# maple3142/gf2bv

Measured on AMD Instinct MI355X. Metric: GF(2) row-XORs/s (solve_one, dense NxN), higher is better.
Workload: dtype u64

## Files before the change

gf2bv_amd/csrc/gf2_kernels.hip.h:

```cpp
#pragma once
#include <hip/hip_runtime.h>
#include <stdint.h>
#include <type_traits>

typedef unsigned long long u64;
typedef long long i64;

#define GF2_GMAX 4
#define GF2_TW 2
#define GF2_TW_LOG 1
#define GF2_LPR 1
#define GF2_OWN_LOG 3
#define GF2_FEW_UNITS 8
#ifndef GF2_BATCH
#define GF2_BATCH 4
#endif
#ifndef GF2_UROWS
#define GF2_UROWS 2
#endif

__device__ __forceinline__ long long tidx(long long row, long long word, long long srows)
{
	return ((word >> GF2_TW_LOG) * srows + row) * GF2_TW + (word & (GF2_TW - 1));
}
struct PanelRec {
	int start;
	int p;
	u64 mask;
};

struct PanelAux {
	int slot_row[64];
	u64 comb[64];
	u64 src_mult[64][GF2_GMAX];
	int first_after;
	int pad;
};

#define GF2_NEVER 0x7f7f7f7f

#define GF2_FEW_MISSING 8
#define GF2_GROUP 16
#define GF2_MAXGROUPS 16

struct SolveState {
	int rank;
	int inconsistent;
	int first;
	unsigned arrive;
	int wide;
	unsigned garr[GF2_MAXGROUPS];
	unsigned claim;
	int self_giveups;
	int fast_off, fast_done;
	int fast_blocks;
	int poison;
	int gate_timeout;
	int fast_pub;
	int sp_chunk;
	int sp_nz;
};

struct SyncFlags {
	int narrow_done;
	int bulk_done;
	unsigned cnt_narrow;
};
struct DoneSignal { unsigned *count; int *flag; int value; };

struct FindUnit {
	u64 have;
	int cnt;
	int first_nonsrc;
	int chunks;
	int pad;
	int srow[64];
	u64 bc[64];
};

__device__ __forceinline__ u64 readlane64(u64 v, int l)
{
	unsigned lo = __builtin_amdgcn_readlane((unsigned)v, l);
	unsigned hi = __builtin_amdgcn_readlane((unsigned)(v >> 32), l);
	return ((u64)hi << 32) | lo;
}
#pragma clang diagnostic push
#pragma clang diagnostic ignored "-Winline-asm"
__device__ __forceinline__ void writelane3(unsigned &d0, unsigned s0, unsigned &d1, unsigned s1, int &d2, int s2, int l)
{
	asm volatile("s_mov_b32 m0, %6\n\tv_writelane_b32 %0, %3, m0\n\tv_writelane_b32 %1, %4, m0\n\tv_writelane_b32 %2, %5, m0"
	             : "+v"(d0), "+v"(d1), "+v"(d2) : "s"(s0), "s"(s1), "s"(s2), "s"(l) : "m0");
}
#pragma clang diagnostic pop
__device__ __forceinline__ int ctz64(u64 v) { return __ffsll((long long)v) - 1; }
__device__ __forceinline__ int uniform(int v) { return __builtin_amdgcn_readfirstlane(v); }
__device__ __forceinline__ u64 lanemask_lt(int lane) { return lane ? (~0ull >> (64 - lane)) : 0ull; }
__device__ __forceinline__ uint4 xor4(uint4 a, uint4 b) { return make_uint4(a.x ^ b.x, a.y ^ b.y, a.z ^ b.z, a.w ^ b.w); }

__host__ __device__ __forceinline__ i64 mult_rows(i64 rows) { return (rows + 63) & ~(i64)63; }
__host__ __device__ __forceinline__ i64 midx(int g, i64 row, i64 rows)
{
	(void)rows;
	return row * 4 + (g ^ (int)((row >> 3) & 1));
}
__device__ __forceinline__ u64 mult_stored(int T, u64 m, i64 row)
{
	(void)T;
	const int sh = 8 * (int)(row & 7);
	return sh ? ((m >> sh) | (m << (64 - sh))) : m;
}
__device__ __forceinline__ u64 mult_plain(int T, u64 v, i64 row)
{
	(void)T;
	const int sh = 8 * (int)(row & 7);
	return sh ? ((v << sh) | (v >> (64 - sh))) : v;
}

struct SysStride { i64 m_words, arena_bytes; };
template <class P>
__device__ __forceinline__ P *sys_at(P *p, i64 bytes)
{
	typedef typename std::remove_cv<P>::type Q;
	return reinterpret_cast<P *>(reinterpret_cast<char *>(const_cast<Q *>(p)) + bytes);
}

__host__ __device__ __forceinline__ i64 owned_item(i64 ct, i64 first, int ulog, int world, int wrank)
{
	if (world <= 1) return first + ct;
	const i64 usz = (i64)1 << ulog;
	const i64 u_first = first >> ulog;
	const i64 u0 = u_first + (((wrank - u_first % world) % world) + world) % world;
	const i64 head = (u0 == u_first) ? usz - (first & (usz - 1)) : 0;
	if (ct < head) return first + ct;
	const i64 c2 = ct - head;
	return ((u0 + ((head ? 1 : 0) + c2 / usz) * world) << ulog) + c2 % usz;
}

__global__ void k_pack_digits(const uint32_t *__restrict__ digits, const i64 *__restrict__ off,
                              int bpd, i64 rows, i64 cols, i64 wtot, i64 srows, u64 *__restrict__ M, SysStride ss, i64 dig_base)
{
	off += blockIdx.z * rows;
	M += blockIdx.z * ss.m_words;
	const i64 w = (i64)blockIdx.x * blockDim.x + threadIdx.x;
	if (w >= wtot) return;
	for (i64 r = blockIdx.y; r < rows; r += gridDim.y) {
	const uint32_t *d = digits + (off[r] - dig_base);
	i64 nd = off[r + 1] - off[r];
	u64 val = 0;
	i64 c0 = w * 64;
	if (c0 < cols) {
		i64 p0 = c0 + 1;
		i64 di = p0 / bpd;
		int sh = (int)(p0 % bpd);
		int filled = 0;
		while (filled < 64 && di < nd) {
			u64 piece = (u64)(d[di] >> sh);
			val |= piece << filled;
			filled += bpd - sh;
			sh = 0;
			di++;
		}
		if (cols - c0 < 64) val &= (1ull << (cols - c0)) - 1;
	}
	if (w == (cols >> 6) && nd > 0) val |= (u64)(d[0] & 1u) << (cols & 63);
	M[tidx(r, w, srows)] = val;
	}
}

__global__ void __launch_bounds__(256)
k_to_tiled(const u64 *__restrict__ src, i64 stride, i64 rows, i64 ntiles, i64 wt, i64 srows, u64 *__restrict__ dst,
           i64 src_sys_words, SysStride ss)
{
	static_assert(GF2_TW == 2, "16-byte tiles");
	src += blockIdx.z * src_sys_words;
	dst += blockIdx.z * ss.m_words;
	__shared__ uint4 buf[16 * 65];
	const int t = threadIdx.x;
	const i64 row0 = (i64)blockIdx.x * 64, tile0 = (i64)blockIdx.y * 16;
	const bool even = ((stride & 1) == 0) && ((reinterpret_cast<size_t>(src) & 15) == 0);
#pragma unroll
	for (int i = 0; i < 4; i++) {
		const int r = (t >> 4) + 16 * i, c = t & 15;
		const i64 row = row0 + r, w = (tile0 + c) * 2;
		uint4 v = make_uint4(0, 0, 0, 0);
		if (row < rows && w < wt) {
			const u64 *p = src + row * stride + w;
			if (even && w + 1 < wt) v = *reinterpret_cast<const uint4 *>(p);
			else {
				const u64 a = p[0], b2 = (w + 1 < wt) ? p[1] : 0ull;
				v = make_uint4((unsigned)a, (unsigned)(a >> 32), (unsigned)b2, (unsigned)(b2 >> 32));
			}
		}
		buf[c * 65 + r] = v;
	}
	__syncthreads();
#pragma unroll
	for (int i = 0; i < 4; i++) {
		const int c = (t >> 6) + 4 * i, r = t & 63;
		const i64 row = row0 + r, tile = tile0 + c;
		if (row < rows && tile < ntiles) reinterpret_cast<uint4 *>(dst)[tile * srows + row] = buf[c * 65 + r];
	}
}


__global__ void __launch_bounds__(256)
k_win_gather(const u64 *__restrict__ M, i64 rows, i64 srows, int j0, int gb, u64 *__restrict__ Wb, const SolveState *__restrict__ st, SysStride ss)
{
	if (sys_at(st, blockIdx.y * ss.arena_bytes)->poison) return;
	M += blockIdx.y * ss.m_words;
	Wb = sys_at(Wb, blockIdx.y * ss.arena_bytes);
	const i64 t = (i64)blockIdx.x * blockDim.x + threadIdx.x;
	const i64 i = t / gb;
	const int g = (int)(t % gb);
	if (i >= rows) return;
	Wb[i * GF2_GMAX + g] = M[tidx(i, j0 + g, srows)];
}

__global__ void __launch_bounds__(256)
k_win_scatter(u64 *__restrict__ M, i64 rows, i64 srows, int j0, int gb, const u64 *__restrict__ Wb,
              const int *__restrict__ died, const SolveState *__restrict__ st, SysStride ss)
{
	M += blockIdx.y * ss.m_words;
	Wb = sys_at(Wb, blockIdx.y * ss.arena_bytes);
	died = sys_at(died, blockIdx.y * ss.arena_bytes);
	if (sys_at(st, blockIdx.y * ss.arena_bytes)->poison) return;
	const i64 t = (i64)blockIdx.x * blockDim.x + threadIdx.x;
	const i64 i = t / gb;
	const int g = (int)(t % gb);
	if (i >= rows || died[i] != GF2_NEVER) return;
	M[tidx(i, j0 + g, srows)] = Wb[i * GF2_GMAX + g];
}

#define GF2_ST(ptr, val) __hip_atomic_store((ptr), (val), __ATOMIC_RELAXED, __HIP_MEMORY_SCOPE_AGENT)
#define GF2_LD(ptr) __hip_atomic_load((ptr), __ATOMIC_RELAXED, __HIP_MEMORY_SCOPE_AGENT)

#define GF2_GATE_TICKS 500000000ull
__global__ void k_probe_wait(int *flag, int *result, unsigned long long ticks)
{
	const unsigned long long t0 = wall_clock64();
	int ok = 0;
	while (!(ok = GF2_LD(flag)) && wall_clock64() - t0 < ticks) __builtin_amdgcn_s_sleep(2);
	*result = ok ? 1 : 2;
}
__global__ void k_probe_set(int *flag) { GF2_ST(flag, 1); }
__global__ void __launch_bounds__(512) k_probe_hold_bulk(unsigned long long *stamp, unsigned long long ticks)
{
	__shared__ unsigned big[133 * 256];
	big[threadIdx.x] = threadIdx.x;
	__syncthreads();
	const unsigned long long t0 = wall_clock64();
	if (blockIdx.x == 0 && threadIdx.x == 0) *stamp = t0;
	while (wall_clock64() - t0 < ticks) __builtin_amdgcn_s_sleep(8);
	if (big[(threadIdx.x + 1) & 511] == 0xffffffffu) *stamp = 0;
}
__global__ void __launch_bounds__(256) k_probe_panel_work(unsigned long long *stamp, unsigned long long ticks)
{
	__shared__ unsigned mid[23 * 256];
	mid[threadIdx.x] = threadIdx.x;
	__syncthreads();
	const unsigned long long t0 = wall_clock64();
	while (wall_clock64() - t0 < ticks) __builtin_amdgcn_s_sleep(4);
	if (threadIdx.x == 0) *stamp = wall_clock64();
	if (mid[(threadIdx.x + 1) & 255] == 0xffffffffu) *stamp = 0;
}
__global__ void __launch_bounds__(256) k_probe_stamp_panel(unsigned long long *stamp)
{
	__shared__ unsigned mid[23 * 256];
	mid[threadIdx.x] = threadIdx.x;
	__syncthreads();
	if (threadIdx.x == 0) *stamp = wall_clock64();
	if (mid[(threadIdx.x + 1) & 255] == 0xffffffffu) *stamp = 0;
}
__global__ void __launch_bounds__(64)
k_probe_xcc(int *out)
{
	if (threadIdx.x == 0) out[blockIdx.x] = (int)(__builtin_amdgcn_s_getreg(20 | (0 << 6) | (3 << 11)) & 15u);
}
__global__ void __launch_bounds__(64)
k_gate(SyncFlags *__restrict__ sf, SolveState *__restrict__ st, int set_narrow, int set_bulk, int need_narrow, int need_bulk,
       SysStride ss)
{
	sf = sys_at(sf, blockIdx.y * ss.arena_bytes); st = sys_at(st, blockIdx.y * ss.arena_bytes);
	if (threadIdx.x != 0) return;
	if (set_narrow > 0) GF2_ST(&sf->narrow_done, set_narrow);
	if (set_bulk > 0) GF2_ST(&sf->bulk_done, set_bulk);
	const unsigned long long t0 = wall_clock64();
	int polls = 0;
	while (GF2_LD(&sf->narrow_done) < need_narrow || GF2_LD(&sf->bulk_done) < need_bulk) {
		if (++polls < 512) __builtin_amdgcn_s_sleep(2); else __builtin_amdgcn_s_sleep(64);
		if (wall_clock64() - t0 > GF2_GATE_TICKS || GF2_LD(&st->gate_timeout)) { GF2_ST(&st->gate_timeout, 1); break; }
	}
}
__device__ __forceinline__ void signal_light(DoneSignal sig, i64 arena_off, unsigned total_wgs)
{
	if (!sig.count) return;
	asm volatile("s_waitcnt vmcnt(0)" ::: "memory");
	__builtin_amdgcn_fence(__ATOMIC_RELEASE, "workgroup");
	__syncthreads();
	if (threadIdx.x == 0) {
		unsigned *cnt = sys_at(sig.count, arena_off);
		const unsigned old = __hip_atomic_fetch_add(cnt, 1u, __ATOMIC_RELAXED, __HIP_MEMORY_SCOPE_AGENT);
		if (old + 1 == total_wgs) { GF2_ST(cnt, 0u); GF2_ST(sys_at(sig.flag, arena_off), sig.value); }
	}
}

#ifdef GF2_STEP_PROBE
#define GF2_PROBE_WGS 384
#define GF2_PROBE_UNITS 256
__device__ int gf2_probe_j0 = -1;
__device__ unsigned long long gf2_probe_wg[GF2_GMAX + 1][GF2_PROBE_WGS][4];
__device__ unsigned long long gf2_probe_un[GF2_GMAX + 1][GF2_PROBE_UNITS][6];
__device__ unsigned long long gf2_probe_gj[4];
__device__ unsigned long long gf2_probe_fast[32];
__device__ unsigned long long gf2_probe_upd[GF2_PROBE_WGS][6];
__device__ unsigned long long gf2_probe_wave[5][16];
#define GF2_PROBE_WG(k) do { if (probe_on && threadIdx.x == 0 && blockIdx.x < GF2_PROBE_WGS) gf2_probe_wg[probe_step][blockIdx.x][k] = wall_clock64(); } while (0)
#define GF2_PROBE_UN(k) do { if (gf2_probe_on_u && lane == 0 && u < GF2_PROBE_UNITS) gf2_probe_un[gf2_probe_step_u][u][k] = wall_clock64(); } while (0)
#define GF2_PROBE_UNV(k, v) do { if (gf2_probe_on_u && lane == 0 && u < GF2_PROBE_UNITS) gf2_probe_un[gf2_probe_step_u][u][k] = (v); } while (0)
#else
#define GF2_PROBE_WG(k) do { } while (0)
#define GF2_PROBE_UN(k) do { } while (0)
#define GF2_PROBE_UNV(k, v) do { } while (0)
#endif

struct FindState {
	u64 bw, bc, have;
	int nslots;
	bool colslots;
	int srow;
};

__device__ __forceinline__ unsigned wave_or32(unsigned x)
{
	x |= (unsigned)__builtin_amdgcn_update_dpp(0, (int)x, 0x111, 0xf, 0xf, false);
	x |= (unsigned)__builtin_amdgcn_update_dpp(0, (int)x, 0x112, 0xf, 0xf, false);
	x |= (unsigned)__builtin_amdgcn_update_dpp(0, (int)x, 0x114, 0xf, 0xf, false);
	x |= (unsigned)__builtin_amdgcn_update_dpp(0, (int)x, 0x118, 0xf, 0xf, false);
	x |= (unsigned)__builtin_amdgcn_update_dpp(0, (int)x, 0x142, 0xa, 0xf, false);
	x |= (unsigned)__builtin_amdgcn_update_dpp(0, (int)x, 0x143, 0xc, 0xf, false);
	return (unsigned)__builtin_amdgcn_readlane((int)x, 63);
}
__device__ __forceinline__ u64 wave_or(u64 v)
{
	return ((u64)wave_or32((unsigned)(v >> 32)) << 32) | wave_or32((unsigned)v);
}
__device__ __forceinline__ unsigned wave_xor32(unsigned x)
{
	x ^= (unsigned)__builtin_amdgcn_update_dpp(0, (int)x, 0x111, 0xf, 0xf, false);
	x ^= (unsigned)__builtin_amdgcn_update_dpp(0, (int)x, 0x112, 0xf, 0xf, false);
	x ^= (unsigned)__builtin_amdgcn_update_dpp(0, (int)x, 0x114, 0xf, 0xf, false);
	x ^= (unsigned)__builtin_amdgcn_update_dpp(0, (int)x, 0x118, 0xf, 0xf, false);
	x ^= (unsigned)__builtin_amdgcn_update_dpp(0, (int)x, 0x142, 0xa, 0xf, false);
	x ^= (unsigned)__builtin_amdgcn_update_dpp(0, (int)x, 0x143, 0xc, 0xf, false);
	return (unsigned)__builtin_amdgcn_readlane((int)x, 63);
}
__device__ __forceinline__ u64 wave_xor(u64 v)
{
	return ((u64)wave_xor32((unsigned)(v >> 32)) << 32) | wave_xor32((unsigned)v);
}

template <class IDX>
__device__ __forceinline__ u64 xor_over_bits(const u64 *base, u64 bits, IDX idx)
{
	u64 acc = 0;
	while (bits) {
		const int b0 = ctz64(bits); bits &= bits - 1;
		const u64 h1 = bits ? ~0ull : 0ull; const int b1 = bits ? ctz64(bits) : b0; bits &= bits - 1;
		const u64 h2 = bits ? ~0ull : 0ull; const int b2 = bits ? ctz64(bits) : b0; bits &= bits - 1;
		const u64 h3 = bits ? ~0ull : 0ull; const int b3 = bits ? ctz64(bits) : b0; bits &= bits - 1;
		const u64 v0 = base[idx(b0)], v1 = base[idx(b1)], v2 = base[idx(b2)], v3 = base[idx(b3)];
		acc ^= v0 ^ (v1 & h1) ^ (v2 & h2) ^ (v3 & h3);
	}
	return acc;
}

__device__ __forceinline__ u64 xor_and64(u64 x, u64 v, unsigned m)
{
	const unsigned lo = (unsigned)__builtin_amdgcn_bitop3_b32((int)(unsigned)x, (int)(unsigned)v, (int)m, 0x78);
	const unsigned hi = (unsigned)__builtin_amdgcn_bitop3_b32((int)(unsigned)(x >> 32), (int)(unsigned)(v >> 32), (int)m, 0x78);
	return ((u64)hi << 32) | lo;
}
template <bool HI>
__device__ __forceinline__ unsigned halfbit_mask(u64 x, int bb)
{
	return (unsigned)__builtin_amdgcn_sbfe((int)(unsigned)(HI ? (x >> 32) : x), (unsigned)bb, 1u);
}

template <int K>
__device__ __forceinline__ u64 transpose_stage(u64 x, int lane)
{
	constexpr u64 mk = K == 32 ? 0x00000000ffffffffull : K == 16 ? 0x0000ffff0000ffffull : K == 8 ? 0x00ff00ff00ff00ffull
	                 : K == 4 ? 0x0f0f0f0f0f0f0f0full : K == 2 ? 0x3333333333333333ull : 0x5555555555555555ull;
	auto partner = [&](unsigned v) -> unsigned {
		if (K == 1) return (unsigned)__builtin_amdgcn_update_dpp(0, (int)v, 0xb1, 0xf, 0xf, false);
		if (K == 2) return (unsigned)__builtin_amdgcn_update_dpp(0, (int)v, 0x4e, 0xf, 0xf, false);
		if (K == 8) return (unsigned)__builtin_amdgcn_update_dpp(0, (int)v, 0x128, 0xf, 0xf, false);
		if (K == 4) {
			const int a = __builtin_amdgcn_update_dpp(0, (int)v, 0x104, 0xf, 0x5, false);
			return (unsigned)__builtin_amdgcn_update_dpp(a, (int)v, 0x114, 0xf, 0xa, false);
		}
		return (unsigned)__builtin_amdgcn_ds_bpermute((lane ^ K) << 2, (int)v);
	};
	const u64 pv = ((u64)partner((unsigned)(x >> 32)) << 32) | partner((unsigned)x);
	return (lane & K) ? ((x & ~mk) | ((pv >> K) & mk)) : ((x & mk) | ((pv << K) & ~mk));
}
__device__ __forceinline__ u64 wave_transpose64(u64 x, int lane)
{
	x = transpose_stage<32>(x, lane); x = transpose_stage<16>(x, lane); x = transpose_stage<8>(x, lane);
	x = transpose_stage<4>(x, lane); x = transpose_stage<2>(x, lane); x = transpose_stage<1>(x, lane);
	return x;
}

__device__ __forceinline__ u64 gj_columns(FindState &S, u64 w, int row, int lane)
{
#ifdef GF2_STEP_PROBE
	const bool gjp = gf2_probe_j0 >= 0 && blockIdx.x == 0 && blockIdx.y == 0 && threadIdx.x == 0;
	if (gjp) gf2_probe_gj[0] = wall_clock64();
#endif
	u64 col = wave_transpose64(w, lane);
#ifdef GF2_STEP_PROBE
	if (gjp) gf2_probe_gj[1] = wall_clock64();
#endif
	u64 used = 0, have = 0;
	int Lv = 0;
	for (int b = 0; b < 64; b++) {
		const u64 v = readlane64(col, b);
		const u64 a = v & ~used;
		if (!a) continue;
		const int L = ctz64(a);
		used |= 1ull << L; have |= 1ull << b;
		const u64 vm = v & ~(1ull << L);
		const unsigned mk = 0u - (unsigned)((col >> L) & 1);
		col = xor_and64(col, vm, mk);
		unsigned clo = (unsigned)col, chi = (unsigned)(col >> 32);
		writelane3(clo, (unsigned)v, chi, (unsigned)(v >> 32), Lv, L, b);
		col = ((u64)chi << 32) | clo;
	}
#ifdef GF2_STEP_PROBE
	if (gjp) gf2_probe_gj[2] = wall_clock64();
#endif
	const u64 rows_t = wave_transpose64(col, lane);
// ... 1362 lines not shown
		comb[g] = aux[j0 + gc].comb[r];
#pragma unroll
		for (int e = 0; e < GF2_GMAX; e++) smul[g][e] = (e < g) ? aux[j0 + gc].src_mult[r][e] : 0ull;
		mrow[g] = multset[midx(gc, ic, rows)];
		if (g >= gb) { rec[g].p = 0; rec[g].mask = 0; mrow[g] = 0; }
	}
	u64 wv[W];
#pragma unroll
	for (int e = 0; e < W; e++) wv[e] = M[tidx(ic, wlo + (e < gnext ? e : 0), srows)];
	const int my_died = wmask ? died[ic] : 0;
	if (blockIdx.x != 0 && (i64)(blockIdx.x + 1) * 256 <= first) {
		if (wmask && (t & 63) == 0 && (i >> 6) < mask_words) { wmask[i >> 6] = 0; wmask[mask_words + (i >> 6)] = 0; }
		return;
	}
	int anyp = 0;
#pragma unroll
	for (int g = 0; g < GF2_GMAX; g++) anyp |= rec[g].p;
	if (anyp) {
#pragma unroll
		for (int g = 0; g < GF2_GMAX; g++) {
			const u64 v = M[tidx(r < rec[g].p ? srow[g] : 0, wlo + (live ? w : 0), srows)];
			S[(g * 64 + r) * W + w] = (r < rec[g].p && live) ? v : 0ull;
			if (w == 0 && ((rec[g].mask >> r) & 1)) Bk[g * 64 + __popcll(rec[g].mask & lanemask_lt(r))] = r;
		}
		__syncthreads();
		auto build_tables = [&](const u64 *rows64) {
			const int n = t >> 4, v = t & 15;
			u64 a[W] = { 0, 0, 0, 0 };
#pragma unroll
			for (int k = 0; k < 4; k++) {
				const u64 on = ((v >> k) & 1) ? ~0ull : 0ull;
#pragma unroll
				for (int e = 0; e < W; e++) a[e] ^= rows64[(4 * n + k) * W + e] & on;
			}
#pragma unroll
			for (int e = 0; e < W; e++) Tn[(n * 16 + v) * W + e] = a[e];
		};
#pragma unroll
		for (int g = 0; g < GF2_GMAX; g++) {
			if (g >= gb) break;
			build_tables(&S[g * 64 * W]);
			__syncthreads();
			if (!((rec[g].mask >> r) & 1)) Pbit[(g * 64 + r) * W + w] = 0;
			if (r < rec[g].p) {
				const u64 acc = nibble_word(Tn, comb[g], w);
				Pbit[(g * 64 + Bk[g * 64 + r]) * W + w] = acc;
				if (blockIdx.x == 0 && live) Uwin[(i64)(rec[g].start + r) * GF2_GMAX + w] = acc;
			}
			__syncthreads();
			build_tables(&Pbit[g * 64 * W]);
			__syncthreads();
#pragma unroll
			for (int h = g + 1; h < GF2_GMAX; h++)
				if (h < gb && r < rec[h].p) S[(h * 64 + r) * W + w] ^= nibble_word(Tn, smul[h][g], w);
			if (i < rows && mrow[g]) {
				u64 acc[W];
				nibble_rows(Tn, mult_plain(upd_T, mrow[g], ic), acc);
#pragma unroll
				for (int e = 0; e < W; e++) wv[e] ^= acc[e];
			}
			__syncthreads();
		}
	}
	if (wmask) {
		u64 any = 0;
#pragma unroll
		for (int e = 0; e < W; e++) if (e < gnext) any |= wv[e];
		const bool alive = i < rows && my_died == GF2_NEVER;
		const u64 ba = __ballot(alive), bn = __ballot(alive && any != 0);
		if ((t & 63) == 0 && (i >> 6) < mask_words) { wmask[i >> 6] = ba; wmask[mask_words + (i >> 6)] = bn; }
	}
	if (i >= rows) return;
#pragma unroll
	for (int e = 0; e < W; e++)
		if (e < gnext) Wb_out[i * GF2_GMAX + e] = wv[e];
}

__global__ void __launch_bounds__(256)
k_window_masks(const u64 *__restrict__ Wb, i64 rows, int gb, const int *__restrict__ died, u64 *__restrict__ wmask, const SolveState *__restrict__ st, SysStride ss)
{
	{
		const i64 ao = blockIdx.y * ss.arena_bytes;
		Wb = sys_at(Wb, ao); died = sys_at(died, ao); wmask = sys_at(wmask, ao); st = sys_at(st, ao);
	}
	if (st->poison) return;
	const i64 mask_words = (rows + 63) >> 6;
	const i64 i = (i64)blockIdx.x * 256 + threadIdx.x, ic = i < rows ? i : rows - 1;
	u64 any = 0;
	for (int e = 0; e < gb; e++) any |= Wb[ic * GF2_GMAX + e];
	const bool alive = i < rows && died[ic] == GF2_NEVER;
	const u64 ba = __ballot(alive), bn = __ballot(alive && any != 0);
	if ((threadIdx.x & 63) == 0 && (i >> 6) < mask_words) { wmask[i >> 6] = ba; wmask[mask_words + (i >> 6)] = bn; }
}

__global__ void __launch_bounds__(256)
k_unwind(u64 *__restrict__ M, i64 srows, int G, int npanels, int nblocks, const SolveState *__restrict__ st,
         const int *__restrict__ pivcol, const int *__restrict__ urow, const u64 *__restrict__ Uwin, int world, int wrank,
         int tl_K, int tl_bend, SysStride ss)
{
	{
		const i64 ao = blockIdx.y * ss.arena_bytes;
		M += blockIdx.y * ss.m_words;
		st = sys_at(st, ao); pivcol = sys_at(pivcol, ao); urow = sys_at(urow, ao); Uwin = sys_at(Uwin, ao);
	}
	const i64 t = (i64)blockIdx.x * blockDim.x + threadIdx.x;
	const i64 k = t / GF2_GMAX;
	const int e = (int)(t % GF2_GMAX);
	if (k >= st->rank) return;
	const int b = (pivcol[k] >> 6) / G;
	if (b + 1 >= nblocks) return;
	if (tl_K > 0 && b < tl_bend && (b + 1) % tl_K == 0) return;
	const int wlo = (b + 1) * G;
	const int gnext = (npanels - wlo < G) ? npanels - wlo : G;
	if (world > 1 && ((wlo + e) >> GF2_OWN_LOG) % world != wrank) return;
	if (e < gnext) M[tidx(urow[k], wlo + e, srows)] = Uwin[k * GF2_GMAX + e];
}

struct SlabSeg { const void *src; void *dst; unsigned bytes; };
struct SlabSegs { SlabSeg s[5]; };
__global__ void __launch_bounds__(256)
k_slab_copy(SlabSegs segs)
{
	const size_t tid = (size_t)blockIdx.x * blockDim.x + threadIdx.x, nth = (size_t)gridDim.x * blockDim.x;
#pragma unroll
	for (int k = 0; k < 5; k++) {
		const SlabSeg g = segs.s[k];
		if (!g.bytes) continue;
		if (((g.bytes | (unsigned)(size_t)g.src | (unsigned)(size_t)g.dst) & 15u) == 0) {
			const uint4 *a = static_cast<const uint4 *>(g.src); uint4 *b = static_cast<uint4 *>(g.dst);
			for (size_t i = tid; i < g.bytes / 16; i += nth) b[i] = a[i];
		} else {
			const unsigned *a = static_cast<const unsigned *>(g.src); unsigned *b = static_cast<unsigned *>(g.dst);
			for (size_t i = tid; i < g.bytes / 4; i += nth) b[i] = a[i];
		}
	}
}

__global__ void __launch_bounds__(256)
k_import_marks(int j0, int gb, const PanelRec *__restrict__ panels, const PanelAux *__restrict__ aux,
               int *__restrict__ died, int *__restrict__ pivcol, int *__restrict__ urow)
{
	const int g = threadIdx.x >> 6, lane = threadIdx.x & 63;
	if (g >= gb) return;
	const PanelRec rec = panels[j0 + g];
	if ((rec.mask >> lane) & 1) pivcol[rec.start + __popcll(rec.mask & lanemask_lt(lane))] = 64 * (j0 + g) + lane;
	if (lane < rec.p) {
		const int sr = aux[j0 + g].slot_row[lane];
		urow[rec.start + lane] = sr;
		died[sr] = j0 + g;
	}
}


template <int TW, int WPW>
__global__ void __launch_bounds__(64 * WPW)
k_block_trsm(u64 *__restrict__ M, i64 srows, int j0, int gb, int wlo, int group_begin, int world, int wrank,
             const PanelRec *__restrict__ panels, const PanelAux *__restrict__ aux, int nw_lo, int nw_hi, u64 *__restrict__ Pc,
             SysStride ss)
{
	__builtin_amdgcn_s_setprio(2);
	M += blockIdx.y * ss.m_words;
	panels = sys_at(panels, blockIdx.y * ss.arena_bytes);
	aux = sys_at(aux, blockIdx.y * ss.arena_bytes);
	if (Pc) Pc = sys_at(Pc, blockIdx.y * ss.arena_bytes);
	constexpr int NT = 64 * WPW;
	static_assert(WPW == 4 && NT == 256, "thread <-> table entry mapping below");
	__shared__ u64 S[GF2_GMAX * 64 * WPW];
	__shared__ u64 Pbit[GF2_GMAX * 64 * WPW];
	__shared__ u64 Tn[16 * 16 * WPW];
	__shared__ int Bk[GF2_GMAX * 64];
	const i64 w0 = owned_item(blockIdx.x, group_begin, GF2_OWN_LOG - 2, world, wrank) * WPW;
	const int t = threadIdx.x;
	const int r = t / WPW, w = t % WPW;
	auto at = [&](i64 row) -> u64 & { return M[tidx(row, w0 + w, srows)]; };
	const bool live = w0 + w >= wlo && !(w0 + w >= nw_lo && w0 + w < nw_hi);
	PanelRec rec[GF2_GMAX];
	int srow[GF2_GMAX];
	u64 comb[GF2_GMAX], smul[GF2_GMAX][GF2_GMAX];
#pragma unroll
	for (int g = 0; g < GF2_GMAX; g++) {
		const int gc = g < gb ? g : 0;
		rec[g] = panels[j0 + gc];
		srow[g] = aux[j0 + gc].slot_row[r];
		comb[g] = aux[j0 + gc].comb[r];
#pragma unroll
		for (int e = 0; e < GF2_GMAX; e++) smul[g][e] = (e < g) ? aux[j0 + gc].src_mult[r][e] : 0ull;
		if (g >= gb) { rec[g].p = 0; rec[g].mask = 0; }
	}
#pragma unroll
	for (int g = 0; g < GF2_GMAX; g++) {
		const u64 v = at(r < rec[g].p ? srow[g] : 0);
		S[(g * 64 + r) * WPW + w] = (r < rec[g].p && live) ? v : 0ull;
		Pbit[(g * 64 + r) * WPW + w] = 0;
		if (w == 0 && ((rec[g].mask >> r) & 1)) Bk[g * 64 + __popcll(rec[g].mask & lanemask_lt(r))] = r;
	}
	__syncthreads();
	auto build_tables = [&](const u64 *rows64) {
		const int n = t >> 4, v = t & 15;
		u64 a[WPW] = { 0, 0, 0, 0 };
#pragma unroll
		for (int k = 0; k < 4; k++) {
			const u64 on = ((v >> k) & 1) ? ~0ull : 0ull;
#pragma unroll
			for (int e = 0; e < WPW; e++) a[e] ^= rows64[(4 * n + k) * WPW + e] & on;
		}
#pragma unroll
		for (int e = 0; e < WPW; e++) Tn[(n * 16 + v) * WPW + e] = a[e];
	};
	auto lookup = [&](u64 m) {
		u64 acc = 0;
#pragma unroll
		for (int n = 0; n < 16; n++) {
			const unsigned half = n < 8 ? (unsigned)m : (unsigned)(m >> 32);
			acc ^= Tn[(n * 16 + ((half >> (4 * (n & 7))) & 15u)) * WPW + w];
		}
		return acc;
	};
#pragma unroll
	for (int g = 0; g < GF2_GMAX; g++) {
		if (g >= gb) break;
		build_tables(&S[g * 64 * WPW]);
		__syncthreads();
		if (r < rec[g].p) {
			const u64 acc = lookup(comb[g]);
			Pbit[(g * 64 + Bk[g * 64 + r]) * WPW + w] = acc;
			if (live) at(srow[g]) = acc;
		}
		if (g + 1 >= gb) break;
		__syncthreads();
		build_tables(&Pbit[g * 64 * WPW]);
		__syncthreads();
#pragma unroll
		for (int h = g + 1; h < GF2_GMAX; h++)
			if (h < gb && r < rec[h].p) S[(h * 64 + r) * WPW + w] ^= lookup(smul[h][g]);
		__syncthreads();
	}
	if (Pc) {
		__syncthreads();
		const i64 wabs = w0 + w;
#pragma unroll
		for (int g = 0; g < GF2_GMAX; g++)
			Pc[(((wabs >> 1) * GF2_GMAX + g) * 64 + r) * 2 + (wabs & 1)] = Pbit[(g * 64 + r) * WPW + w];
	}
	(void)NT;
}

__host__ __device__ __forceinline__ int mult_slot(int g, i64 row) { return g ^ (int)((row >> 3) & 1); }
__host__ __device__ __forceinline__ u64 mult_rot(u64 m, i64 row)
{
	const int sh = 8 * (int)(row & 7);
	return sh ? ((m >> sh) | (m << (64 - sh))) : m;
}
__host__ __device__ __forceinline__ u64 mult_unrot(u64 m, i64 row)
{
	const int sh = 8 * (int)(row & 7);
	return sh ? ((m << sh) | (m >> (64 - sh))) : m;
}

typedef unsigned u32x4 __attribute__((ext_vector_type(4)));
typedef __attribute__((address_space(3))) const u32x4 *lds_u4_ptr;

template <int NT, bool HALF, int DEPTH, bool PIPE, int LB, bool STREAM = false>
__global__ void __launch_bounds__(LB)
k_update16(u64 *__restrict__ M, i64 rows, i64 srows, int j0, int gb, int wlo,
           const PanelRec *__restrict__ panels, const PanelAux *__restrict__ aux,
           const u64 *__restrict__ mult4, const int *__restrict__ blk_first,
           int tile_begin, int ntiles, int world, int wrank, const uint4 *__restrict__ Pc, SysStride ss, int xcd_nsys)
{
	unsigned bx = blockIdx.x, gx = gridDim.x, by = blockIdx.y;
	if (xcd_nsys > 0) {
		const unsigned slot = bx >> 3, xcd = bx & 7;
		gx = gx / (unsigned)xcd_nsys;
		by = (slot / gx) * 8 + xcd;
		bx = slot % gx;
	}
	{
		const i64 ao = (i64)by * ss.arena_bytes;
		M += (i64)by * ss.m_words;
		panels = sys_at(panels, ao); aux = sys_at(aux, ao); mult4 = sys_at(mult4, ao); blk_first = sys_at(blk_first, ao);
		if (Pc) Pc = sys_at(Pc, ao);
	}
	constexpr int NW = NT / 64;
	__shared__ __attribute__((aligned(256))) uint4 tab[2 * 256 * 16];
	__shared__ uint4 stage[GF2_GMAX * 64];
	__shared__ int prow[GF2_GMAX * 64];
	const int lane = threadIdx.x & 63, wv = threadIdx.x >> 6;
	if ((unsigned)(size_t)tab != 0u) __builtin_trap();

	int anyp = 0;
	for (int g = 0; g < gb; g++) anyp |= panels[j0 + g].p;
	if (!anyp) return;
	const i64 rlo = (i64)(*blk_first) & ~(i64)63;
	const i64 R64 = (rows + 63) & ~(i64)63;
	constexpr int ALIGN = NW * 64;
	const i64 R = (R64 - rlo + ALIGN - 1) / ALIGN * ALIGN;
	const i64 total = (i64)ntiles * R;
	i64 chunk = (total + gx - 1) / gx;
	chunk = (chunk + ALIGN - 1) / ALIGN * ALIGN;
	i64 pos = (i64)bx * chunk;
	const i64 pend = (pos + chunk < total) ? pos + chunk : total;

	unsigned KC[6];
	{
		const int rq_lo = lane & 7, rq_hi = (lane >> 3) & 1;
#pragma unroll
		for (int v = 0; v < 6; v++) {
			unsigned k = 1u << 24;
#pragma unroll
			for (int b = 0; b < 3; b++) {
				const int s = 3 * v + b;
				if (s < 16) k |= (unsigned)(16 * (8 * ((s >> 3) ^ rq_hi) + (((s & 7) + rq_lo) & 7))) << (8 * b);
			}
			asm volatile("" : "+v"(k));
			KC[v] = k;
		}
	}

	unsigned sgx = 0, sgy = 0, sgz = 0, sgw = 0;
	bool have_staged = false;
	for (bool first_span = true; pos < pend; first_span = false) {
		const int ct = (int)(pos / R);
		const i64 r0 = pos - (i64)ct * R;
		const i64 span = (R - r0 < pend - pos) ? R - r0 : pend - pos;
		pos += span;
		const i64 tile = owned_item(ct, tile_begin, GF2_OWN_LOG - 1, world, wrank);
		const i64 rbeg = rlo + r0;
		if (rbeg >= R64) continue;
		const i64 rend = (rbeg + span < R64) ? rbeg + span : R64;
		uint4 *Mw = reinterpret_cast<uint4 *>(M) + tile * srows;
		const uint4 *mq = reinterpret_cast<const uint4 *>(mult4);
		const i64 nsteps = (rend - rbeg + ALIGN - 1) / ALIGN;
		i64 nb = nsteps;
		if (rbeg + ((nsteps - 1) * NW + wv) * 64 >= rend) nb--;
		struct Bt { uint4 d, m0, m1; i64 row; };
		auto load = [&](Bt &H, i64 i) {
			const i64 ic = i < nb ? i : nb - 1;
			const i64 row = rbeg + (ic * NW + wv) * 64 + lane;
			H.row = row;
			H.m0 = mq[row * 2]; H.m1 = mq[row * 2 + 1];
#ifdef GF2_MB_L2
			H.d = Mw[row & 4095];
#elif defined(GF2_NT_LOAD)
			{ const u32x4 t = __builtin_nontemporal_load(reinterpret_cast<const u32x4 *>(Mw + row)); H.d = make_uint4(t.x, t.y, t.z, t.w); }
#else
			if (STREAM) { const u32x4 t = __builtin_nontemporal_load(reinterpret_cast<const u32x4 *>(Mw + row)); H.d = make_uint4(t.x, t.y, t.z, t.w); }
			else H.d = Mw[row];
#endif
		};
		Bt H[DEPTH] = {};
		if (nb > 0) {
#pragma unroll
			for (int d = 0; d < DEPTH - 1; d++) load(H[d], d);
		}
		if (!first_span) __syncthreads();
		if (first_span && !Pc) {
			for (int t = threadIdx.x; t < GF2_GMAX * 64; t += NT) {
				const int g = t >> 6, b = t & 63;
				int pr = -1;
				if (g < gb) {
					const PanelRec rec = panels[j0 + g];
					if ((rec.mask >> b) & 1) pr = aux[j0 + g].slot_row[__popcll(rec.mask & ((1ull << b) - 1))];
				}
				prow[t] = pr;
			}
			__syncthreads();
		}
		const uint4 *Mq = reinterpret_cast<const uint4 *>(M) + tile * srows;
		if (threadIdx.x < GF2_GMAX * 64) {
			const int pr = Pc ? 0 : prow[threadIdx.x];
			uint4 v;
			if (have_staged) { v.x = sgx; v.y = sgy; v.z = sgz; v.w = sgw; }
			else v = Pc ? Pc[tile * (GF2_GMAX * 64) + threadIdx.x] : Mq[pr >= 0 ? pr : 0];
			const bool k0 = pr >= 0 && 2 * tile >= wlo, k1 = pr >= 0 && 2 * tile + 1 >= wlo;
			if (!k0) { v.x = 0; v.y = 0; }
			if (!k1) { v.z = 0; v.w = 0; }
			stage[threadIdx.x] = v;
		}
		__syncthreads();
		for (int it = threadIdx.x; it < 2 * 31 * 16; it += NT) {
			const int sub = it & 15, e = (it >> 4) % 31, grp = (it >> 4) / 31;
			const int idx = e <= 15 ? e : (e - 15) << 4;
			const uint4 *st = stage + (2 * grp + (sub >> 3)) * 64 + 8 * (sub & 7);
			uint4 acc = make_uint4(0, 0, 0, 0);
			int bits = idx;
			while (bits) {
				const int l = __ffs(bits) - 1; bits &= bits - 1;
				acc = xor4(acc, st[l]);
			}
			tab[grp * 4096 + idx * 16 + sub] = acc;
		}
		__syncthreads();
		for (int it = threadIdx.x; it < 2 * 225 * 16; it += NT) {
			const int sub = it & 15, k = (it >> 4) % 225, grp = (it >> 4) / 225;
			const int lo = 1 + k % 15, hi = (1 + k / 15) << 4;
			uint4 *tb = tab + grp * 4096 + sub;
			tb[(lo | hi) * 16] = xor4(tb[lo * 16], tb[hi * 16]);
		}
		__syncthreads();

		have_staged = false;
		if (pos < pend) {
			const i64 ntile = owned_item((int)(pos / R), tile_begin, GF2_OWN_LOG - 1, world, wrank);
			if (threadIdx.x < GF2_GMAX * 64) {
				uint4 nx;
				if (Pc) nx = Pc[ntile * (GF2_GMAX * 64) + threadIdx.x];
				else {
					const int pr = prow[threadIdx.x];
					nx = (reinterpret_cast<const uint4 *>(M) + ntile * srows)[pr >= 0 ? pr : 0];
				}
				sgx = nx.x; sgy = nx.y; sgz = nx.z; sgw = nx.w;
			}
			have_staged = true;
		}
		auto issue = [&](u32x4 *v, const Bt &H, int r) {
			const unsigned mw[8] = { H.m0.x, H.m0.y, H.m0.z, H.m0.w, H.m1.x, H.m1.y, H.m1.z, H.m1.w };
			const int grp = r >> 1, hf = r & 1;
#pragma unroll
			for (int k = 0; k < 8; k++) {
				const int s = 8 * hf + k;
				const unsigned sel = (unsigned)(s % 3) | ((4u + (unsigned)(k & 3)) << 8) | ((grp ? 3u : 12u) << 16) | (12u << 24);
				const unsigned at = __builtin_amdgcn_perm(mw[2 * (2 * grp + hf) + (k >> 2)], KC[s / 3], sel);
				v[k] = *(lds_u4_ptr)(size_t)at;
			}
		};
		auto fold = [&](uint4 &acc, const u32x4 *v) {
#pragma unroll
			for (int h = 0; h < 4; h++) {
				acc.x = __builtin_amdgcn_bitop3_b32(acc.x, v[2 * h].x, v[2 * h + 1].x, 0x96);
				acc.y = __builtin_amdgcn_bitop3_b32(acc.y, v[2 * h].y, v[2 * h + 1].y, 0x96);
				acc.z = __builtin_amdgcn_bitop3_b32(acc.z, v[2 * h].z, v[2 * h + 1].z, 0x96);
				acc.w = __builtin_amdgcn_bitop3_b32(acc.w, v[2 * h].w, v[2 * h + 1].w, 0x96);
			}
		};
		auto store = [&](const Bt &H, const uint4 &acc) {
#ifdef GF2_MB_L2
			const i64 q = H.row & 4095;
#else
			const i64 q = H.row;
#endif
			if (HALF) reinterpret_cast<u64 *>(Mw + q)[1] = ((u64)acc.w << 32) | acc.z;
#ifdef GF2_NT_STORE
			else { const u32x4 t = { acc.x, acc.y, acc.z, acc.w }; __builtin_nontemporal_store(t, reinterpret_cast<u32x4 *>(Mw + q)); }
#else
			else if (STREAM) { const u32x4 t = { acc.x, acc.y, acc.z, acc.w }; __builtin_nontemporal_store(t, reinterpret_cast<u32x4 *>(Mw + q)); }
			else Mw[q] = acc;
#endif
		};
		if (nb > 0) {
			u32x4 va[8], vb[8];
#ifndef GF2_MB_NOLOOKUP
			if (PIPE) issue(va, H[0], 0);
#endif
			for (i64 i = 0; i < nb; i += DEPTH) {
#pragma unroll
				for (int d = 0; d < DEPTH; d++) {
					if (i + d >= nb) break;
					load(H[(d + DEPTH - 1) % DEPTH], i + d + DEPTH - 1);
					Bt &C = H[d];
					uint4 acc = C.d;
#ifdef GF2_MB_NOLOOKUP
					acc.x ^= C.m0.x ^ C.m0.y ^ C.m0.z ^ C.m0.w; acc.y ^= C.m1.x ^ C.m1.y ^ C.m1.z ^ C.m1.w;
#else
					if (PIPE) {
						issue(vb, C, 1); fold(acc, va);
						issue(va, C, 2); fold(acc, vb);
						issue(vb, C, 3); fold(acc, va);
						issue(va, H[(d + 1) % DEPTH], 0); fold(acc, vb);
					} else {
#pragma unroll
						for (int r = 0; r < 4; r++) { issue(va, C, r); fold(acc, va); }
					}
#endif
					store(C, acc);
				}
			}
		}
	}
}


#ifndef GF2_KMAX
#define GF2_KMAX 12
#endif
#ifndef GF2_KSEG
#define GF2_KSEG 16
#endif

template <int WPW, bool IDENT>
__global__ void __launch_bounds__(64 * WPW)
k_outer_trsm(u64 *__restrict__ M, i64 rows, i64 srows, int j0, int npan, int group_begin,
             const PanelRec *__restrict__ panels, const PanelAux *__restrict__ aux,
             const u64 *__restrict__ mult, i64 set_words, int set0, int nsets, int upd_T, u64 *__restrict__ Tm, SysStride ss)
{
	static_assert(WPW == 4, "thread <-> table entry mapping below");
	{
		const i64 ao = blockIdx.y * ss.arena_bytes;
		M += blockIdx.y * ss.m_words;
		panels = sys_at(panels, ao); aux = sys_at(aux, ao); mult = sys_at(mult, ao); Tm = sys_at(Tm, ao);
	}
	constexpr int NP = GF2_KMAX * GF2_GMAX;
	__shared__ u64 S[NP * 64 * WPW];
	__shared__ u64 Pb[64 * WPW];
	__shared__ u64 Tn[16 * 16 * WPW];
	__shared__ int srowL[NP * 64];
	__shared__ int Bk[64];
	__shared__ u64 mL[NP * 64];
	const i64 w0 = ((i64)group_begin + blockIdx.x) * WPW;
	const int t = threadIdx.x, r = t / WPW, w = t % WPW;
	for (int q = w; q < npan; q += WPW) srowL[q * 64 + r] = (r < panels[j0 + q].p) ? aux[j0 + q].slot_row[r] : -1;
	__syncthreads();
	for (int q = 0; q < npan; q++) {
		const int sr = srowL[q * 64 + r];
		if (IDENT) S[(q * 64 + r) * WPW + w] = (sr >= 0 && q == (int)w0 + w) ? (1ull << r) : 0ull;
		else S[(q * 64 + r) * WPW + w] = sr >= 0 ? M[tidx(sr, w0 + w, srows)] : 0ull;
	}
	auto put_T = [&](int q, u64 v) {
		const i64 i = (i64)q * 64 + r;
		Tm[((i64)blockIdx.x * (NP * 64) + i) * GF2_GMAX + (w ^ (int)((i >> 3) & 1))] = mult_stored(upd_T, v, i);
	};
	auto build_tables = [&](const u64 *rows64) {
		const int n = t >> 4, v = t & 15;
		u64 a[WPW] = { 0, 0, 0, 0 };
#pragma unroll
		for (int k = 0; k < 4; k++) {
			const u64 on = ((v >> k) & 1) ? ~0ull : 0ull;
#pragma unroll
			for (int e = 0; e < WPW; e++) a[e] ^= rows64[(4 * n + k) * WPW + e] & on;
		}
#pragma unroll
		for (int e = 0; e < WPW; e++) Tn[(n * 16 + v) * WPW + e] = a[e];
	};
	auto lookup = [&](u64 m) {
		u64 acc = 0;
#pragma unroll
		for (int n = 0; n < 16; n++) {
			const unsigned half = n < 8 ? (unsigned)m : (unsigned)(m >> 32);
			acc ^= Tn[(n * 16 + ((half >> (4 * (n & 7))) & 15u)) * WPW + w];
		}
		return acc;
	};
	constexpr int MPT = NP * 64 / (64 * WPW);
	u64 mreg[MPT];
	auto fetch_mults = [&](int q) {
		const int g = q % GF2_GMAX, blk = q / GF2_GMAX;
		const u64 *mset = mult + (i64)((set0 + blk) % nsets) * set_words;
#pragma unroll
		for (int u = 0; u < MPT; u++) {
			const int i = t + u * 64 * WPW;
			u64 m = 0;
			if (i < (npan - q - 1) * 64) {
				const int q2 = q + 1 + i / 64, sl = i % 64;
				const int row2 = srowL[q2 * 64 + sl];
				if (row2 >= 0) m = (q2 / GF2_GMAX == blk) ? aux[j0 + q2].src_mult[sl][g] : mult_plain(upd_T, mset[midx(g, row2, rows)], row2);
			}
			mreg[u] = m;
		}
	};
	auto put_mults = [&](int q) {
#pragma unroll
		for (int u = 0; u < MPT; u++) {
			const int i = t + u * 64 * WPW;
			if (i < (npan - q - 1) * 64) mL[(q + 1 + i / 64) * 64 + i % 64] = mreg[u];
		}
	};
	fetch_mults(0);
	put_mults(0);
	__syncthreads();
	for (int q = 0; q < npan; q++) {
		const PanelRec rec = panels[j0 + q];
		if (q + 1 < npan) fetch_mults(q + 1);
		if (rec.p != 0) {
			const u64 comb = aux[j0 + q].comb[r];
			build_tables(&S[q * 64 * WPW]);
			Pb[r * WPW + w] = 0;
			if (w == 0 && ((rec.mask >> r) & 1)) Bk[__popcll(rec.mask & lanemask_lt(r))] = r;
			__syncthreads();
			u64 acc = 0;
			if (r < rec.p) {
				acc = lookup(comb);
				Pb[Bk[r] * WPW + w] = acc;
				if (!IDENT) M[tidx(srowL[q * 64 + r], w0 + w, srows)] = acc;
			}
			if (IDENT) put_T(q, acc);
			__syncthreads();
			if (q + 1 >= npan) break;
			build_tables(Pb);
			__syncthreads();
			for (int q2 = q + 1; q2 < npan; q2++) {
				const u64 m = mL[q2 * 64 + r];
				if (m) S[(q2 * 64 + r) * WPW + w] ^= lookup(m);
			}
		} else if (IDENT) put_T(q, 0ull);
		__syncthreads();
		if (q + 1 < npan) put_mults(q + 1);
		__syncthreads();
	}
}

#define GF2_OUTER_LISTS (2 * GF2_KMAX * GF2_GMAX * 64 + GF2_KMAX)
__global__ void __launch_bounds__(256)
k_outer_prow(int j0, int nblk, const PanelRec *__restrict__ panels, const PanelAux *__restrict__ aux, int *__restrict__ out, SysStride ss)
{
	{
		const i64 ao = blockIdx.y * ss.arena_bytes;
		panels = sys_at(panels, ao); aux = sys_at(aux, ao); out = sys_at(out, ao);
	}
	constexpr int NQ = GF2_KMAX * GF2_GMAX * 64;
	__shared__ int anyb[GF2_KMAX];
	if (threadIdx.x < GF2_KMAX) anyb[threadIdx.x] = 0;
	__syncthreads();
	for (int t = threadIdx.x; t < NQ; t += blockDim.x) {
		int pr = -1, sr = -1;
		if (t < nblk * GF2_GMAX * 64) {
			const int q = t >> 6, b = t & 63;
			const PanelRec rec = panels[j0 + q];
			if ((rec.mask >> b) & 1) { pr = aux[j0 + q].slot_row[__popcll(rec.mask & ((1ull << b) - 1))]; anyb[q / GF2_GMAX] = 1; }
			if (b < rec.p) sr = aux[j0 + q].slot_row[b];
		}
		out[t] = pr;
		out[NQ + GF2_KMAX + t] = sr;
	}
	__syncthreads();
	if (threadIdx.x < GF2_KMAX) out[NQ + threadIdx.x] = anyb[threadIdx.x];
}

template <int SEG, int NT_, int RB, int NB>
__device__ __forceinline__ void
update16k_body(u64 *__restrict__ M, i64 rows, i64 srows, int nblk, const int *__restrict__ gprow,
               const u64 *__restrict__ mult, i64 set_words, int set0, int nsets,
               const int *__restrict__ blk_first, const int *__restrict__ died, int j_end, int tile_begin, int ntiles, SysStride ss,
               int chunk_major)
// ... 2610 lines not shown
```

gf2bv_amd/csrc/gf2_solver.hip:

```cpp
#include "gf2_kernels.hip.h"
#include <hip/hip_ext.h>
#include "../../include/gf2bv_hip.h"

#include <algorithm>
#include <array>
#include <atomic>
#include <chrono>
#include <cstdio>
#include <cstdlib>
#include <cstring>
#include <functional>
#include <map>
#include <memory>
#include <new>
#include <mutex>
#include <string>
#include <thread>
#include <unordered_map>
#include <vector>

namespace {

thread_local std::string g_err = "";

// ... 269 lines not shown
		std::lock_guard<std::mutex> lk(mu);
		auto &v = events[{device, timing ? 1 : 0}];
		if (v.size() < 8192) v.push_back(e); else (void)hipEventDestroy(e);
	}
	hipError_t stream(hipStream_t *s, int device, int cls)
	{
		const bool low = cls & 1;
		{
			std::lock_guard<std::mutex> lk(mu);
			auto &v = streams[{device, cls}];
			if (!v.empty()) { *s = v.back(); v.pop_back(); return hipSuccess; }
		}
		if (!low) return hipStreamCreateWithFlags(s, hipStreamNonBlocking);
		int lo = 0, hi = 0;
		(void)hipDeviceGetStreamPriorityRange(&lo, &hi);
		return hipStreamCreateWithPriority(s, hipStreamNonBlocking, lo);
	}
	void release_stream(hipStream_t s, int device, int cls)
	{
		if (!s) return;
		std::lock_guard<std::mutex> lk(mu);
		streams[{device, cls}].push_back(s);
	}
	static constexpr int kMaxLow = 10;
	std::mutex probe_mu;
	std::map<std::pair<hipStream_t, hipStream_t>, int> pair_ok;
	std::map<int, int> low_created;
	int pairs_probed = 0, pairs_bad = 0;
	hipError_t probe_pair(hipStream_t a, hipStream_t b, int device, int *ok, const Knobs &kn, int depth = 0)
	{
		*ok = 1;
		constexpr int NB = 6;
		unsigned long long *q = nullptr, hq[2 * NB + 2];
		int *fl = nullptr;
		hipError_t e = alloc((void **)&q, sizeof hq, device);
		if (e != hipSuccess) return e;
		struct Free { Pool *p; void *q; ~Free() { p->release(q); } } g1{ this, q };
		if ((e = alloc((void **)&fl, sizeof(int) * 2 * NB, device)) != hipSuccess) return e;
		Free g2{ this, fl };
		if ((e = hipMemsetAsync(fl, 0, sizeof(int) * 2 * NB, a)) != hipSuccess) return e;
		if ((e = hipMemsetAsync(q, 0, sizeof hq, a)) != hipSuccess) return e;
		if ((e = hipStreamSynchronize(a)) != hipSuccess) return e;
		if ((e = hipStreamSynchronize(b)) != hipSuccess) return e;
		int cus = 256;
		(void)hipDeviceGetAttribute(&cus, hipDeviceAttributeMultiprocessorCount, device);
		k_probe_stamp_panel<<<dim3(1), dim3(256), 0, a>>>(q + 2 * NB);
		for (int i = 0; i < NB; i++) {
			k_probe_panel_work<<<dim3(1), dim3(256), 0, a>>>(q + 2 * i, 1000ull);
			k_probe_panel_work<<<dim3(1), dim3(256), 0, a>>>(q + 2 * i + 1, 1000ull);
			k_probe_set<<<dim3(1), dim3(1), 0, a>>>(fl + i);
			k_probe_wait<<<dim3(1), dim3(1), 0, b>>>(fl + i, fl + NB + i, 200000ull);
			k_probe_hold_bulk<<<dim3((unsigned)cus), dim3(512), 0, b>>>(q + 2 * NB + 1, 4000ull);
		}
		if ((e = hipGetLastError()) != hipSuccess) return e;
		if ((e = hipStreamSynchronize(a)) != hipSuccess) return e;
		if ((e = hipStreamSynchronize(b)) != hipSuccess) return e;
		if ((e = hipMemcpy(hq, q, sizeof hq, hipMemcpyDeviceToHost)) != hipSuccess) return e;
		const double chain_us = ((double)hq[2 * NB - 1] - (double)hq[2 * NB]) / 100.0;
		*ok = chain_us < 37.0 * NB;
		if (depth < 2 && chain_us > 0.75 * 37.0 * NB && chain_us < 1.5 * 37.0 * NB) {
			int again = 1;
			if (probe_pair(a, b, device, &again, kn, depth + 1) == hipSuccess) *ok = *ok || again;
		}
		if (kn.trace)
			fprintf(stderr, "[gf2bv trace] stream pair %p / %p: the panel chain of %d probe blocks took %.1f us (%s)\n", (void *)a, (void *)b, NB, chain_us,
			        *ok ? "good" : "waits for the bulk stream");
		return hipSuccess;
	}
	hipError_t low_stream_for(const Knobs &kn, hipStream_t a, int device, hipStream_t *out, int cls = 1, const std::vector<hipStream_t> &also = {})
	{
		if (!(kn.stream_pairs >= 0 ? kn.stream_pairs != 0 : !kn.plain) || !a) return stream(out, device, cls);
		std::lock_guard<std::mutex> pl(probe_mu);
		std::vector<hipStream_t> rejected, with;
		with.push_back(a);
		for (hipStream_t x : also) if (x && x != a) with.push_back(x);
		hipError_t err = hipSuccess;
		*out = nullptr;
		auto known = [&](hipStream_t c) {
			int r = 1;
			for (hipStream_t x : with) {
				auto it = pair_ok.find({x, c});
				if (it == pair_ok.end()) r = r == 0 ? 0 : -1; else if (it->second == 0) r = 0;
			}
			return r;
		};
		for (int attempt = 0; attempt < kMaxLow + 2 && !*out; attempt++) {
			hipStream_t c = nullptr;
			bool known_good = false;
			{
				std::lock_guard<std::mutex> lk(mu);
				auto &v = streams[{device, cls}];
				for (size_t i = v.size(); i-- > 0 && !c;)
					if (known(v[i]) == 1) { c = v[i]; v.erase(v.begin() + (ptrdiff_t)i); known_good = true; }
				for (size_t i = v.size(); i-- > 0 && !c;)
					if (known(v[i]) == -1) { c = v[i]; v.erase(v.begin() + (ptrdiff_t)i); }
				if (!c) {
					if (low_created[device] >= kMaxLow) break;
					low_created[device]++;
				}
			}
			if (known_good) { *out = c; break; }
			if (!c) {
				int lo = 0, hi = 0;
				(void)hipDeviceGetStreamPriorityRange(&lo, &hi);
				if ((err = hipStreamCreateWithPriority(&c, hipStreamNonBlocking, lo)) != hipSuccess) break;
			}
			int all_ok = 1;
			for (hipStream_t x : with) {
				int ok = -1;
				{
					std::lock_guard<std::mutex> lk(mu);
					auto it = pair_ok.find({x, c});
					if (it != pair_ok.end()) ok = it->second;
				}
				if (ok < 0) {
					ok = 1;
					if (probe_pair(x, c, device, &ok, kn) != hipSuccess) { (void)hipGetLastError(); ok = 1; }
					else {
						std::lock_guard<std::mutex> lk(mu);
						pair_ok[{x, c}] = ok;
						pairs_probed++; pairs_bad += !ok;
					}
				}
				if (!ok) { all_ok = 0; break; }
			}
			if (all_ok) *out = c; else rejected.push_back(c);
		}
		if (!*out && !rejected.empty()) { *out = rejected.front(); rejected.erase(rejected.begin()); }
		for (hipStream_t r : rejected) release_stream(r, device, cls);
		if (!*out && err == hipSuccess) return stream(out, device, cls);
		return err;
	}
};
Pool &pool()
{
	static Pool *p = new Pool();
	return *p;
}
int alloc_or_nomem(void **out, size_t bytes, int device, const char *nomem, const char *what)
{
	const hipError_t e = pool().alloc(out, bytes, device);
	if (e == hipErrorOutOfMemory) { (void)hipGetLastError(); return fail(GF2BV_ERR_NOMEM, nomem); }
	if (e != hipSuccess) return fail(GF2BV_ERR_HIP, what, e);
	return GF2BV_OK;
}

int streams_run_concurrently(const Knobs &kn, int device, hipStream_t a, hipStream_t b, int *ok);
int xcd_dispatch_is_round_robin(int device, hipStream_t st, int *ok);
void forget_concurrency(int device);

struct UpdateImpl {
	int G, T, lds_bytes, threads;
	hipError_t (*update)(dim3, hipStream_t, u64 *, i64, i64, int, int, int, const PanelRec *, const PanelAux *,
	                     const u64 *, const int *, int, int, int, int, int, bool, const uint4 *, SysStride, hipEvent_t, hipEvent_t, int);
};

template <int NT, int DEPTH, bool PIPE, int LB>
hipError_t launch_update16(dim3 grid, hipStream_t s, u64 *M, i64 rows, i64 srows, int j0, int gb, int wlo,
                           const PanelRec *panels, const PanelAux *aux, const u64 *multset, const int *blk_first,
                           int tile_begin, int ntiles, int world, int wrank, int nw_lo, bool stream_rows, const uint4 *Pc, SysStride ss,
                           hipEvent_t begun, hipEvent_t done, int xcd_nsys)
{
	if (xcd_nsys > 0) grid = dim3(grid.x * grid.y);
	{
		if (stream_rows && NT == 512 && DEPTH == 3 && PIPE && LB == 512) {
			if (nw_lo < 0)
				hipExtLaunchKernelGGL((k_update16<512, true, 3, true, 512, true>), grid, dim3(512), 0, s, begun, done, 0, M, rows, srows, j0, gb, wlo,
				                      panels, aux, multset, blk_first, tile_begin, ntiles, world, wrank, Pc, ss, xcd_nsys);
			else
				hipExtLaunchKernelGGL((k_update16<512, false, 3, true, 512, true>), grid, dim3(512), 0, s, begun, done, 0, M, rows, srows, j0, gb, wlo,
				                      panels, aux, multset, blk_first, tile_begin, ntiles, world, wrank, Pc, ss, xcd_nsys);
			return hipGetLastError();
		}
	}
	if (nw_lo < 0)
		hipExtLaunchKernelGGL((k_update16<NT, true, DEPTH, PIPE, LB>), grid, dim3(NT), 0, s, begun, done, 0, M, rows, srows, j0, gb, wlo,
		                      panels, aux, multset, blk_first, tile_begin, ntiles, world, wrank, Pc, ss, xcd_nsys);
	else
		hipExtLaunchKernelGGL((k_update16<NT, false, DEPTH, PIPE, LB>), grid, dim3(NT), 0, s, begun, done, 0, M, rows, srows, j0, gb, wlo,
		                      panels, aux, multset, blk_first, tile_begin, ntiles, world, wrank, Pc, ss, xcd_nsys);
	return hipGetLastError();
}
#define UPDATE16_IMPL(NT, D, P, LB) { 4, 8, 2 * 256 * 256 + GF2_GMAX * 64 * 20, NT, launch_update16<NT, D, P, LB> }

const UpdateImpl kUpdates[] = {
	UPDATE16_IMPL(512, 3, true, 512),
	UPDATE16_IMPL(768, 2, true, 768),
	UPDATE16_IMPL(768, 2, true, 1024),
	UPDATE16_IMPL(1024, 2, false, 1024),
	UPDATE16_IMPL(768, 3, true, 768),
	UPDATE16_IMPL(640, 2, true, 640),
};

static_assert(sizeof kUpdates / sizeof kUpdates[0] == Knobs::kNumUpdates, "GF2BV_UPDATE indexes this table");

constexpr int YK = 5, YTW = 16, YNT = 1024;
hipError_t launch_ysweep(dim3 grid, hipStream_t s, u64 *Y, i64 ys, i64 rows, const PanelRec *rec,
                         const u64 *mult, int ntiles, int rpb)
{
	constexpr int lds = SweepCfg<YK, YTW>::LDS_BYTES;
	static std::mutex attr_mu;
	static std::map<int, bool> attr_set;
	int dev = 0;
	(void)hipGetDevice(&dev);
	{
		std::lock_guard<std::mutex> lk(attr_mu);
		if (!attr_set[dev]) {
			hipError_t e = hipFuncSetAttribute((const void *)k_sweep<YK, YTW, YNT>,
			                                   hipFuncAttributeMaxDynamicSharedMemorySize, lds);
			if (e != hipSuccess) return e;
			attr_set[dev] = true;
		}
	}
	k_sweep<YK, YTW, YNT><<<grid, dim3(YNT), lds, s>>>(Y, ys, rows, rec, 1, mult, 0, ntiles, rpb);
	return hipGetLastError();
}

constexpr int TW = GF2_TW;

inline size_t round256(size_t bytes) { return (bytes + 255) & ~(size_t)255; }

struct ArenaLayout {
	size_t st = 0, sf = 0, panels = 0, aux = 0, fu = 0, died = 0, pivcol = 0, urow = 0, blk_first = 0, mult = 0, Wb = 0, Uwin = 0, Pfast = 0,
	       oprow = 0, Tm = 0, Pc = 0, wmask = 0, stride = 0;
};

struct SolverPlan {
	int device = 0;
	i64 rows = 0, cols = 0, stride = 0;
	i64 ntiles = 0, srows = 0;
	int nsys = 1;
	int gang_nsys = 1;
	int world = 1, wrank = 0;
	i64 m_stride = 0, src_sys_words = 0;
	ArenaLayout lay;
	bool view = false;
	bool own_bs = true;
	SysStride ss() const { return SysStride{ m_stride, (i64)lay.stride }; }
	int mode = 0;
	int nrhs = 1;
	bool time_kernels = false;
	Knobs kn;
	const UpdateImpl *impl = nullptr;

	int nsets = 2;
	int tl_K = 0, tl_bend = 0;
	i64 tile_hi = 0;
	static constexpr int nlist = 2;
	bool bulk_waits_outer = false;
	bool ends_outer_panel(int b) const { return tl_K > 0 && b < tl_bend && (b + 1) % tl_K == 0; }
	bool flag_sync = true;
	bool optimistic = true;
	bool xcd_pin = true;
	int sync_base = 0;
	int units = 0;
	bool sparse_on = false;
	int sparse_giveups = 0;
	int sparse_tier = 0;
	int narrow_rpt = 1;
	i64 ys = 0;
	int ny = 0;
	int h_ycol = 0;
	i64 maxr = 0;
	int npanels = 0, nblocks = 0;
	i64 wt = 0, cw = 0;

	std::vector<int> free_order;
	SolveState hst{};
	std::vector<u64> hout;
	std::vector<PanelRec> hp;
	std::vector<int32_t> hpiv;
	std::chrono::steady_clock::time_point t_begin;
	float ms_pack = 0;
};

ArenaLayout arena_layout(const SolverPlan &P)
{
	const i64 R = std::max<i64>(1, P.rows), NP = std::max(1, P.npanels);
	const int G = P.impl->G;
	ArenaLayout L;
	size_t off = 0;
	auto carve = [&](size_t bytes) { size_t at = off; off += round256(bytes); return at; };
	L.st = carve(sizeof(SolveState)); L.sf = carve(sizeof(SyncFlags)); L.panels = carve(sizeof(PanelRec) * NP); L.aux = carve(sizeof(PanelAux) * NP);
	L.fu = carve(sizeof(FindUnit) * (P.units + 1 + GF2_MAXGROUPS)); L.died = carve(sizeof(int) * (size_t)R);
	L.pivcol = carve(sizeof(int) * (P.maxr + 64)); L.urow = carve(sizeof(int) * (P.maxr + 64));
	L.blk_first = carve(sizeof(int) * std::max(1, P.nblocks)); L.mult = carve(sizeof(u64) * P.nsets * G * mult_rows(R) + (P.tl_K ? kOuterSlackBytes : 0));
	L.Wb = carve(sizeof(u64) * 2 * GF2_GMAX * R); L.Uwin = carve(sizeof(u64) * GF2_GMAX * (P.maxr + 64));
	L.Pfast = carve(sizeof(u64) * GF2_GMAX * GF2_GMAX * 64); L.oprow = carve(sizeof(int) * GF2_OUTER_LISTS * P.nlist);
	L.Tm = carve(P.tl_K ? P.nlist * sizeof(u64) * GF2_KMAX * GF2_KMAX * GF2_GMAX * 64 * GF2_GMAX : 0);
	L.Pc = carve(P.kn.pc ? sizeof(u64) * 2 * GF2_GMAX * 64 * (size_t)P.ntiles : 0);
	L.wmask = carve(sizeof(u64) * 2 * (size_t)((R + 63) / 64 + 1));
	L.stride = off;
	return L;
}

struct ArenaPtrs {
	SolveState *st = nullptr;
	SyncFlags *sf = nullptr;
	PanelRec *panels = nullptr;
	PanelAux *aux = nullptr;
	FindUnit *fu = nullptr;
	int *died = nullptr;
	int *pivcol = nullptr, *urow = nullptr, *blk_first = nullptr;
	u64 *mult = nullptr;
	u64 *Wb = nullptr;
	u64 *Uwin = nullptr;
	u64 *Pfast = nullptr;
	int *oprow = nullptr;
	u64 *Tm = nullptr;
	u64 *Pc = nullptr;
	u64 *wmask = nullptr;

	void bind(const ArenaLayout &L, void *arena, bool pc)
	{
		char *base = (char *)arena;
		st = (SolveState *)(base + L.st); sf = (SyncFlags *)(base + L.sf); panels = (PanelRec *)(base + L.panels); aux = (PanelAux *)(base + L.aux);
		fu = (FindUnit *)(base + L.fu); died = (int *)(base + L.died); pivcol = (int *)(base + L.pivcol); urow = (int *)(base + L.urow);
		blk_first = (int *)(base + L.blk_first); mult = (u64 *)(base + L.mult); Wb = (u64 *)(base + L.Wb); Uwin = (u64 *)(base + L.Uwin);
		Pfast = (u64 *)(base + L.Pfast); oprow = (int *)(base + L.oprow); Tm = (u64 *)(base + L.Tm);
		Pc = pc ? (u64 *)(base + L.Pc) : nullptr;
		wmask = (u64 *)(base + L.wmask);
	}
};

struct SolverHandles {
	hipStream_t sA = nullptr, sB = nullptr;
	bool own_sA = false, own_sB = false;
	u64 *M = nullptr;
	bool ext_M = false;
	const u64 *src = nullptr;
	u64 *tmp_src = nullptr;
	u64 *Minv = nullptr;
	u64 *rhs_bad = nullptr;
	void *arena = nullptr;
	hipStream_t sC = nullptr;
	hipEvent_t evOuter = nullptr, evPri = nullptr, evPanelDone = nullptr, evBig = nullptr;
	u64 *Y = nullptr;
	int *ycols = nullptr;
	u64 *out = nullptr;
	hipEvent_t ev0 = nullptr, ev1 = nullptr, ev2 = nullptr, ev3 = nullptr;
	std::vector<hipEvent_t> evA, evPrio, kev, waitPrio;
	hipEvent_t evx = nullptr;
};

struct Solver : SolverPlan, ArenaPtrs, SolverHandles {
	SolverPlan &plan() { return *this; }
	const SolverPlan &plan() const { return *this; }
	Solver() = default;
	Solver(const Solver &) = delete;
	Solver &operator=(const Solver &) = delete;
	~Solver() { release(); }
	void release()
	{
		if (!arena && !M && !tmp_src && !Y && !ycols && !out && !sA && !sB && !ev0) return;
		(void)hipSetDevice(device);
		Pool &P = pool();
		if (view) {
			if (sA && (Y || ycols || out)) (void)hipStreamSynchronize(sA);
			if (own_bs) for (void *p : { (void *)Y, (void *)ycols, (void *)out, (void *)Minv }) P.release(p);
			P.release_event(ev2, true);
			P.release_event(evx, true);
			arena = nullptr; M = nullptr; sA = sB = nullptr; ev0 = ev1 = ev3 = nullptr;
		} else {
			if (sC) (void)hipStreamSynchronize(sC);
			if (sB) (void)hipStreamSynchronize(sB);
			if (arena || M) (void)hipStreamSynchronize(sA);
			for (void *p : { arena, (void *)Y, (void *)ycols, (void *)out, (void *)Minv, (void *)(ext_M ? nullptr : M), (void *)tmp_src }) P.release(p);
			for (hipEvent_t e : { ev0, ev1, ev2, ev3, evx }) P.release_event(e, true);
			for (hipEvent_t e : { evOuter, evPri, evPanelDone, evBig }) P.release_event(e, false);
			if (sC) P.release_stream(sC, device, nsys > 1 ? 3 : 1);
			for (hipEvent_t e : kev) P.release_event(e, true);
			for (hipEvent_t e : evA) P.release_event(e, false);
			for (hipEvent_t e : evPrio) P.release_event(e, false);
			if (own_sB && sB) P.release_stream(sB, device, nsys > 1 ? 3 : 1);
			if (own_sA && sA) P.release_stream(sA, device, false);
		}
		static_cast<ArenaPtrs &>(*this) = ArenaPtrs();
		static_cast<SolverHandles &>(*this) = SolverHandles();
	}
};

}

struct gf2bv_result {
	int status = 0;
	i64 rank = 0, dim = 0, cw = 0;
	std::vector<u64> origin, basis;
	std::vector<int32_t> pivots;
	gf2bv_stats stats{};
};

namespace {

struct Scratch {
	std::vector<void *> bufs;
	std::vector<hipEvent_t> timing_events;
	hipStream_t sync_first = nullptr;
	~Scratch()
	{
		if (sync_first) (void)hipStreamSynchronize(sync_first);
		for (void *p : bufs) pool().release(p);
		for (hipEvent_t e : timing_events) pool().release_event(e, true);
	}
	hipError_t alloc(void **out, size_t bytes, int device)
	{
		hipError_t e = pool().alloc(out, bytes, device);
		if (e == hipSuccess) bufs.push_back(*out);
		return e;
	}
	hipError_t event(hipEvent_t *ev)
	{
		hipError_t e = pool().event(ev, true);
		if (e == hipSuccess) timing_events.push_back(*ev);
		return e;
	}
};

int check_device(int device)
{
	int n = 0;
	hipError_t e = hipGetDeviceCount(&n);
	if (e != hipSuccess || n <= 0)
		return fail(GF2BV_ERR_NODEVICE, "no HIP device visible: gf2bv_amd has no CPU fallback");
	if (device < 0 || device >= n) return fail(GF2BV_ERR_ARG, "device index out of range");
	HIPCHK(hipSetDevice(device));
	return GF2BV_OK;
}

void plan_two_level(Solver &S)
{
	S.tl_K = 0; S.tl_bend = 0; S.nsets = 2;
	if (S.world != 1 || S.ext_M || S.impl->G != GF2_GMAX) return;
	if (S.nsys != 1) return;
	int K = (double)S.rows * (double)S.wt * 8.0 >= 3.0 * 1073741824.0 ? GF2_KMAX : 8;
	double min_bytes = 0.5 * 1073741824.0;
	if (S.kn.two_level == 0) return;
	if (S.kn.two_level > 0) { K = S.kn.two_level; min_bytes = 0; }
	if (S.kn.two_level_min_set) min_bytes = 1048576.0 * S.kn.two_level_min_mib;
	const int G = S.impl->G;
	int bend = 0;
	for (int b0 = 0; b0 + K < S.nblocks; b0 += K) {
		const i64 rows_left = S.rows - (i64)(b0 + K) * 64 * G, words_left = S.wt - (i64)(b0 + K) * G;
		if ((i64)(b0 + K) * 64 * G > S.cols || rows_left <= 0 || words_left <= 0) break;
		if ((double)rows_left * (double)words_left * 8.0 * (double)S.nsys < min_bytes) break;
		bend = b0 + K;
	}
	if (!bend) return;
	S.tl_K = K; S.tl_bend = bend;
	S.nsets = 2 * K;
}

int solver_alloc(Solver &S)
{
	const Knobs &kn = S.kn = Knobs::read();
	S.wt = (S.cols + S.nrhs + 63) / 64;
	S.cw = (S.cols + 63) / 64;
	S.npanels = (int)((S.cols + 63) / 64);
	S.maxr = std::min(S.rows, S.cols);
	S.impl = &kUpdates[S.kn.update];
	S.ntiles = tiles_for(S.wt);
	S.srows = slab_rows(S.rows);
	S.m_stride = S.ntiles * TW * S.srows;
	if (!S.M) HIPCHK(pool().alloc((void **)&S.M, sizeof(u64) * S.m_stride * S.nsys + kOuterSlackBytes, S.device));
	if (S.src && S.rows > 0) {
		k_to_tiled<<<dim3((unsigned)((S.rows + 63) / 64), (unsigned)((S.ntiles + 15) / 16), S.nsys), dim3(256), 0, S.sA>>>(
			S.src, S.stride, S.rows, S.ntiles, std::min(S.wt, S.stride), S.srows, S.M, S.src_sys_words, S.ss());
	}
	const int G = S.impl->G;
	S.nblocks = (S.npanels + G - 1) / G;
	S.tile_hi = S.ntiles;
	plan_two_level(S);
	S.units = (int)std::min<i64>(256, std::max<i64>(1, (S.rows + 255) / 256));
	S.flag_sync = S.world == 1 && !kn.plain && kn.flag_sync != 0 && !kn.serial;
	S.optimistic = kn.optimistic >= 0 ? kn.optimistic != 0 : !kn.plain;
	S.xcd_pin = kn.xcd_pin >= 0 ? kn.xcd_pin != 0 : !kn.plain;
	if (kn.xcd_pin < 0 && !kn.plain && S.nsys >= 8 && S.nsys % 8 == 0) {
		int ok = 0;
		int rc = xcd_dispatch_is_round_robin(S.device, S.sA, &ok);
		if (rc) return rc;
		S.xcd_pin = ok != 0;
	}
	{
		const i64 blocks = (S.rows + 255) / 256 * std::max(1, S.nsys);
		S.narrow_rpt = (int)std::min<i64>(8, std::max<i64>(1, blocks / 256));
	}
	if (kn.serial) { S.sB = S.sA; S.own_sB = false; }
	else {
		if (S.nsys == 1) HIPCHK(pool().low_stream_for(kn, S.sA, S.device, &S.sB));
		else HIPCHK(pool().stream(&S.sB, S.device, 3));
		S.own_sB = true;
	}
	if (S.flag_sync && S.sB != S.sA) {
		int ok = 0;
		int rc = streams_run_concurrently(kn, S.device, S.sA, S.sB, &ok);
		if (rc) return rc;
		S.flag_sync = ok != 0;
	}
	{
		const ArenaLayout &L = S.lay = arena_layout(S);
		S.sync_base = 0;
		HIPCHK(pool().alloc(&S.arena, L.stride * S.nsys, S.device));
		S.bind(L, S.arena, kn.pc);
		for (int s = 0; s < S.nsys; s++) {
			char *b = (char *)S.arena + (size_t)s * L.stride;
			HIPCHK(hipMemsetAsync(b + L.st, 0, L.died - L.st, S.sA));
			HIPCHK(hipMemsetAsync(b + L.died, GF2_NEVER & 0xff, sizeof(int) * (size_t)std::max<i64>(1, S.rows), S.sA));
			HIPCHK(hipMemsetAsync(b + L.blk_first, 0, L.Wb - L.blk_first, S.sA));
		}
	}
	HIPCHK(pool().event(&S.ev0, true));
	HIPCHK(pool().event(&S.ev1, true));
	HIPCHK(pool().event(&S.ev2, true));
	HIPCHK(pool().event(&S.ev3, true));
	if (S.tl_K) {
		for (hipEvent_t *e : { &S.evOuter, &S.evPri, &S.evPanelDone }) HIPCHK(pool().event(e, false));
		if (S.sB != S.sA) { if (S.nsys == 1) HIPCHK(pool().low_stream_for(kn, S.sA, S.device, &S.sC)); else HIPCHK(pool().stream(&S.sC, S.device, 3)); }
		HIPCHK(pool().event(&S.evBig, false));
	}
	S.evA.resize(S.nblocks); S.evPrio.resize(S.nblocks); S.waitPrio.assign(S.nblocks, nullptr);
	for (int b = 0; b < S.nblocks; b++) {
		HIPCHK(pool().event(&S.evA[b], false));
		HIPCHK(pool().event(&S.evPrio[b], false));
	}
	return GF2BV_OK;
}

struct ConcurrencyCache { std::mutex mu; std::map<int, int> known; };
ConcurrencyCache &concurrency_cache() { static ConcurrencyCache c; return c; }
void forget_concurrency(int device)
{
	ConcurrencyCache &c = concurrency_cache();
	std::lock_guard<std::mutex> lk(c.mu);
	c.known[device] = 0;
}
int streams_run_concurrently(const Knobs &kn, int device, hipStream_t a, hipStream_t b, int *ok)
{
	std::mutex &mu = concurrency_cache().mu;
	std::map<int, int> &known = concurrency_cache().known;
	std::lock_guard<std::mutex> lk(mu);
	auto it = known.find(device);
	if (it != known.end()) { *ok = it->second; return GF2BV_OK; }
	if (kn.flag_sync == 2) { *ok = 1; return GF2BV_OK; }
	int *d = nullptr;
	HIPCHK(pool().alloc((void **)&d, 2 * sizeof(int), device));
	struct Free { int *p; ~Free() { pool().release(p); } } guard{d};
	HIPCHK(hipMemsetAsync(d, 0, 2 * sizeof(int), a));
	HIPCHK(hipStreamSynchronize(a));
	HIPCHK(hipStreamSynchronize(b));
	k_probe_wait<<<dim3(1), dim3(1), 0, a>>>(d, d + 1, 200000ull);
	k_probe_set<<<dim3(1), dim3(1), 0, b>>>(d);
	HIPCHK(hipGetLastError());
	HIPCHK(hipStreamSynchronize(a));
	HIPCHK(hipStreamSynchronize(b));
	int h[2] = { 0, 0 };
	HIPCHK(hipMemcpy(h, d, sizeof h, hipMemcpyDeviceToHost));
	*ok = known[device] = (h[1] == 1);
	return GF2BV_OK;
}

int xcd_dispatch_is_round_robin(int device, hipStream_t st, int *ok)
{
	static std::mutex mu;
	static std::map<int, int> known;
	std::lock_guard<std::mutex> lk(mu);
	auto it = known.find(device);
	if (it != known.end()) { *ok = it->second; return GF2BV_OK; }
	int *d = nullptr;
	HIPCHK(pool().alloc((void **)&d, 64 * sizeof(int), device));
	struct Free { int *p; ~Free() { pool().release(p); } } guard{d};
	int h[64];
	int good = 1;
	for (int rep = 0; rep < 2 && good; rep++) {
		k_probe_xcc<<<dim3(64), dim3(64), 0, st>>>(d);
		HIPCHK(hipGetLastError());
		HIPCHK(hipMemcpyAsync(h, d, sizeof h, hipMemcpyDeviceToHost, st));
		HIPCHK(hipStreamSynchronize(st));
		for (int b = 0; b < 64; b++) if (h[b] != h[b & 7]) good = 0;
		for (int a = 0; a < 8; a++) for (int b = a + 1; b < 8; b++) if (h[a] == h[b]) good = 0;
	}
	*ok = known[device] = good;
	return GF2BV_OK;
}

int pick_update_wgs(i64 est_rows, int ntiles, int nsys, int pinned_wgs = 0)
{
	i64 want = 256;
	want = std::max<i64>(1, want / std::max(1, nsys));
	if (pinned_wgs > 0) want = pinned_wgs;
	constexpr i64 min_rows = 2048;
	const i64 cap = std::max<i64>(1, (i64)ntiles * TW / 8 * est_rows / min_rows);
	return (int)std::min(want, cap);
}

i64 owned_count(i64 first, i64 end, int ulog, int world, int wrank)
{
	if (end <= first) return 0;
	if (world <= 1) return end - first;
	i64 n = 0;
	for (i64 u = first >> ulog; u <= (end - 1) >> ulog; u++)
		if (u % world == wrank) n += std::min<i64>(end, (u + 1) << ulog) - std::max<i64>(first, u << ulog);
	return n;
}

int launch_trsm(Solver &S, hipStream_t st, int j0, int gb, int wlo, int nw_lo, int nw_hi)
{
	constexpr int WPW = 4;
	const i64 g0 = wlo / WPW, g1 = S.tile_hi * TW / WPW;
	const i64 ng = owned_count(g0, g1, GF2_OWN_LOG - 2, S.world, S.wrank);
	if (ng <= 0) return GF2BV_OK;
	k_block_trsm<TW, WPW><<<dim3((unsigned)ng, S.nsys), dim3(64 * WPW), 0, st>>>(S.M, S.srows, j0, gb, wlo, (int)g0, S.world, S.wrank,
	                                                                           S.panels, S.aux, nw_lo, nw_hi, S.Pc, S.ss());
	HIPCHK(hipGetLastError());
	return GF2BV_OK;
}

int launch_update_timed(Solver &S, hipStream_t st, int b, int j0, int gb, int wlo, u64 *mset, int tile_begin, int ntiles,
                        int nw_lo, bool last, hipEvent_t *handoff)
{
	hipEvent_t ka = nullptr, kb = nullptr;
	if (S.time_kernels) {
		HIPCHK(pool().event(&ka, true)); HIPCHK(pool().event(&kb, true));
		S.kev.push_back(ka); S.kev.push_back(kb);
	}
	const i64 est_rows = std::max<i64>(256, S.rows - (i64)j0 * 64);
	const bool pin = S.xcd_pin && S.nsys >= 8 && S.nsys % 8 == 0;
	const int wgs = pick_update_wgs(est_rows, ntiles, S.nsys, pin ? S.kn.xcd_wgs : 0);
	const hipEvent_t begun = ka, done = S.time_kernels ? kb : (last && !S.flag_sync ? S.evPrio[b] : nullptr);
	HIPCHK(S.impl->update(dim3((unsigned)wgs, S.nsys), st, S.M, S.rows, S.srows, j0, gb, wlo, S.panels, S.aux, mset,
	                      S.blk_first + b, tile_begin, ntiles, S.world, S.wrank, nw_lo, pin && S.kn.gang_nt,
	                      (const uint4 *)S.Pc, S.ss(), begun, done, pin ? S.nsys : 0));
	if (last && !S.flag_sync) *handoff = done;
	return GF2BV_OK;
}

struct BlockGeom { int j0, gb, wlo, tb, nt_all, gnext; u64 *mset; };
BlockGeom block_geom(const Solver &S, int b)
{
	const int G = S.impl->G;
	BlockGeom g;
	g.j0 = b * G;
	g.gb = std::min(G, S.npanels - g.j0);
	g.wlo = g.j0 + g.gb;
	g.mset = S.mult + (i64)(b % S.nsets) * G * mult_rows(S.rows);
	g.tb = g.wlo / TW;
	g.nt_all = (g.wlo < S.wt) ? (int)S.tile_hi - g.tb : 0;
	g.gnext = (b + 1 < S.nblocks && !S.ends_outer_panel(b)) ? std::min(G, S.npanels - g.wlo) : 0;
	return g;
}

bool fast_block_possible(const Solver &S, const BlockGeom &g)
{
	return S.kn.fast && g.gb == GF2_GMAX && (i64)(g.j0 + g.gb) * 64 <= S.cols && S.rows >= GF2_FAST_NC;
}

int panel_handover(Solver &S, int b)
{
	k_gate<<<dim3(1, S.nsys), dim3(64), 0, S.sA>>>(S.sf, S.st, S.sync_base + b + 1, 0, 0, 0, S.ss());
	HIPCHK(hipGetLastError());
	return GF2BV_OK;
}

constexpr int kSparseByDensity = 2;
int enqueue_block_panel(Solver &S, int b, bool fast_only = false, bool sparse = false)
{
	const BlockGeom g = block_geom(S, b);
	const unsigned row_blocks = (unsigned)((S.rows + 255) / 256);
	u64 *const half[2] = { S.Wb, S.Wb + (i64)GF2_GMAX * S.rows };
	const hipEvent_t done = S.flag_sync ? nullptr : S.evA[b];
	const DoneSignal sig = S.flag_sync ? DoneSignal{ &S.sf->cnt_narrow, &S.sf->narrow_done, S.sync_base + b + 1 } : DoneSignal{};
	if (fast_only && !sparse && S.kn.fused_narrow && S.nsys == 1) {
		const int rpt = (int)std::min<i64>(8, std::max<i64>(S.narrow_rpt, (row_blocks + 127) / 128));
		hipExtLaunchKernelGGL(k_block_fast_narrow, dim3(1 + (row_blocks + rpt - 1) / rpt, S.nsys), dim3(256), 0, S.sA, nullptr, done, 0,
		                      S.M, S.rows, S.srows, g.j0, g.gb, b, (const u64 *)half[0], S.st, S.died, S.panels, S.aux, S.pivcol, S.urow,
		                      S.blk_first + b, S.Pfast, g.mset, S.impl->T, rpt, sig, S.ss());
		HIPCHK(hipGetLastError());
		return GF2BV_OK;
	}
	if (fast_only) {
		if (!sparse)
			k_block_fast<<<dim3(1, S.nsys), dim3(256), 0, S.sA>>>(S.M, S.rows, S.srows, g.j0, g.gb, 1, b, (const u64 *)half[0], S.st, S.died,
			                                                      S.panels, S.aux, S.pivcol, S.urow, S.blk_first + b, S.Pfast, S.ss());
		else if (S.sparse_tier == 0)
			k_block_sparse<256, 4><<<dim3(1, S.nsys), dim3(256), 0, S.sA>>>(S.M, S.rows, S.srows, g.j0, g.gb, 1, b, (const u64 *)half[0], S.st, S.died,
			                                                                 S.panels, S.aux, S.pivcol, S.urow, S.blk_first + b, (const u64 *)S.wmask, S.ss());
		else if (S.sparse_tier == 1)
			k_block_sparse<512, 8><<<dim3(1, S.nsys), dim3(512), 0, S.sA>>>(S.M, S.rows, S.srows, g.j0, g.gb, 1, b, (const u64 *)half[0], S.st, S.died,
			                                                                S.panels, S.aux, S.pivcol, S.urow, S.blk_first + b, (const u64 *)S.wmask, S.ss());
		else
			k_block_sparse<1024, 6><<<dim3(1, S.nsys), dim3(1024), 0, S.sA>>>(S.M, S.rows, S.srows, g.j0, g.gb, 1, b, (const u64 *)half[0], S.st, S.died,
			                                                                  S.panels, S.aux, S.pivcol, S.urow, S.blk_first + b, (const u64 *)S.wmask, S.ss());
		hipExtLaunchKernelGGL(k_narrow_all, dim3((row_blocks + S.narrow_rpt - 1) / S.narrow_rpt, S.nsys), dim3(256), 0, S.sA, nullptr, done, 0,
		                      (const u64 *)S.M, S.rows, S.srows, g.j0, b, (const u64 *)half[0], (const SolveState *)S.st, (const int *)S.died,
		                      (const PanelAux *)S.aux, g.mset, S.impl->T, S.narrow_rpt, sig, S.ss());
		HIPCHK(hipGetLastError());
		return GF2BV_OK;
	}
	if (fast_block_possible(S, g))
		k_block_fast<<<dim3(1, S.nsys), dim3(256), 0, S.sA>>>(S.M, S.rows, S.srows, g.j0, g.gb, 0, b, (const u64 *)half[0], S.st, S.died,
		                                                      S.panels, S.aux, S.pivcol, S.urow, S.blk_first + b, S.Pfast, S.ss());
	for (int s = 0; s <= g.gb; s++) {
		const int gp = s - 1, gf = (s < g.gb) ? s : -1;
		const i64 c0 = (i64)(g.j0 + std::max(gf, 0)) * 64;
		const u64 colmask = (S.cols - c0 >= 64) ? ~0ull : ((1ull << (S.cols - c0)) - 1);
		const int find_wgs = gf >= 0 ? (S.units + 3) / 4 : 0;
		const unsigned wgs = (unsigned)find_wgs + (gp >= 0 ? (row_blocks + S.narrow_rpt - 1) / S.narrow_rpt : 0u);
		const bool ext = !S.flag_sync && s == g.gb && b != S.nblocks - 1;
		hipExtLaunchKernelGGL(k_panel_step, dim3(wgs, S.nsys), dim3(256), 0, S.sA, nullptr, ext ? S.evA[b] : nullptr, 0,
		                      S.M, S.rows, S.srows, g.j0, gp, gf, g.gb, colmask,
		                      (const u64 *)half[s ? (s - 1) & 1 : 0], half[s & 1], S.st, S.died, S.fu, S.units, find_wgs,
		                      S.panels, S.aux, S.pivcol, S.urow, g.mset,
		                      gf == g.gb - 1 ? S.blk_first + b : (int *)nullptr, S.impl->T, kSparseByDensity, S.kn.self_wait_us * 100, S.narrow_rpt, b, S.ss());
	}
	if (b == S.nblocks - 1)
		k_win_scatter<<<dim3((unsigned)((S.rows * g.gb + 255) / 256), S.nsys), dim3(256), 0, S.sA>>>(S.M, S.rows, S.srows, g.j0, g.gb, half[g.gb & 1], S.died, S.st, S.ss());
	HIPCHK(hipGetLastError());
	if (S.flag_sync) { int rc = panel_handover(S, b); if (rc) return rc; }
	else if (b == S.nblocks - 1) HIPCHK(hipEventRecord(S.evA[b], S.sA));
	if (S.kn.debug_sync & 1) HIPCHK(hipDeviceSynchronize());
	return GF2BV_OK;
}

int enqueue_block_bulk(Solver &S, int b)
{
	const BlockGeom g = block_geom(S, b);
	if (S.bulk_waits_outer) { HIPCHK(hipStreamWaitEvent(S.sB, S.evOuter, 0)); S.bulk_waits_outer = false; }
	if (S.flag_sync) {
		k_gate<<<dim3(1, S.nsys), dim3(64), 0, S.sB>>>(S.sf, S.st, 0, S.sync_base + b, S.sync_base + b + 1, 0, S.ss());
		HIPCHK(hipGetLastError());
	} else HIPCHK(hipStreamWaitEvent(S.sB, S.evA[b], 0));
	bool launched = false;
	if (g.nt_all > 0) {
		int rc = launch_trsm(S, S.sB, g.j0, g.gb, g.wlo, g.wlo, g.wlo + g.gnext);
		if (rc) return rc;
		const int wend = g.wlo + g.gnext;
		const int tfull = g.gnext > 0 ? (wend + 1) / 2 : g.wlo / 2;
		const i64 nfull = owned_count(tfull, S.tile_hi, GF2_OWN_LOG - 1, S.world, S.wrank);
		if ((wend & 1) && g.gnext > 0 && owned_count(wend / 2, wend / 2 + 1, GF2_OWN_LOG - 1, S.world, S.wrank) > 0) {
			rc = launch_update_timed(S, S.sB, b, g.j0, g.gb, g.wlo, g.mset, wend / 2, 1, -1, nfull <= 0, &S.waitPrio[b]);
			if (rc) return rc;
			launched = nfull <= 0;
		}
		if (nfull > 0) {
			rc = launch_update_timed(S, S.sB, b, g.j0, g.gb, g.wlo, g.mset, tfull, (int)nfull, 0, true, &S.waitPrio[b]);
			if (rc) return rc;
			launched = true;
		}
	}
	if (!launched && !S.flag_sync) {
		HIPCHK(hipEventRecord(S.evPrio[b], S.sB));
		S.waitPrio[b] = S.evPrio[b];
	}
	if (S.kn.debug_sync & 2) HIPCHK(hipDeviceSynchronize());
	return GF2BV_OK;
}

int enqueue_block_prio(Solver &S, int b)
{
	if (b + 1 >= S.nblocks || S.ends_outer_panel(b)) return GF2BV_OK;
	const BlockGeom g = block_geom(S, b);
	const unsigned row_blocks = (unsigned)((S.rows + 255) / 256);
	if (b > 0 && !S.flag_sync) HIPCHK(hipStreamWaitEvent(S.sA, S.waitPrio[b - 1], 0));
	if (b > 0 && S.flag_sync) {
		k_gate<<<dim3(1, S.nsys), dim3(64), 0, S.sA>>>(S.sf, S.st, 0, 0, 0, S.sync_base + b, S.ss());
		HIPCHK(hipGetLastError());
	}
	k_prio_window<<<dim3(row_blocks, S.nsys), dim3(256), 0, S.sA>>>(S.M, S.rows, S.srows, g.j0, g.gb, g.wlo, std::max(g.gnext, 1),
	                                                             S.panels, S.aux, g.mset, S.blk_first + b, S.Wb, S.Uwin,
	                                                             S.impl->T, S.st, S.ss(), (const int *)S.died, S.sparse_on ? S.wmask : (u64 *)nullptr);
	HIPCHK(hipGetLastError());
	return GF2BV_OK;
}

int enqueue_forward_begin(Solver &S, bool gather_first_window)
{
	HIPCHK(hipEventRecord(S.ev0, S.sA));
	HIPCHK(hipStreamWaitEvent(S.sB, S.ev0, 0));
	if (S.npanels > 0 && gather_first_window) {
		const int g0 = std::min(S.impl->G, S.npanels);
		k_win_gather<<<dim3((unsigned)((S.rows * g0 + 255) / 256), S.nsys), dim3(256), 0, S.sA>>>(S.M, S.rows, S.srows, 0, g0, S.Wb, S.st, S.ss());
	}
	return GF2BV_OK;
}

int enqueue_forward_join(Solver &S)
{
	HIPCHK(hipEventRecord(S.ev3, S.sB));
	HIPCHK(hipStreamWaitEvent(S.sA, S.ev3, 0));
	if (S.nblocks > 1 && S.maxr > 0)
		k_unwind<<<dim3((unsigned)((S.maxr * GF2_GMAX + 255) / 256), S.nsys), dim3(256), 0, S.sA>>>(
			S.M, S.srows, S.impl->G, S.npanels, S.nblocks, S.st, S.pivcol, S.urow, S.Uwin, S.world, S.wrank, S.tl_K, S.tl_bend, S.ss());
	HIPCHK(hipGetLastError());
	return GF2BV_OK;
}

int enqueue_check_rhs(Solver &S)
{
	int g = (int)std::min<i64>(1024, (S.rows + 255) / 256);
	if (S.rhs_bad) {
		const i64 nrw = ((S.cols & 63) + S.nrhs + 63) / 64;
		k_check_rhs_many<<<dim3(g, (unsigned)std::min<i64>(nrw, 65535)), dim3(256), 0, S.sA>>>(S.M, S.rows, S.srows, S.cols, S.nrhs,
		                                                                                      S.died, S.rhs_bad);
	} else {
		k_check_rhs<<<dim3(g, S.nsys), dim3(256), 0, S.sA>>>(S.M, S.rows, S.srows, S.cols, S.died, S.st, S.ss());
	}
	HIPCHK(hipGetLastError());
	HIPCHK(hipEventRecord(S.ev1, S.sA));
	return GF2BV_OK;
}

int enqueue_outer_prepare(Solver &S, hipStream_t st, int b0, int b1)
{
	const int G = S.impl->G;
	const i64 set_words = (i64)G * mult_rows(S.rows);
	const int npan = (b1 - b0) * G;
	int *gprow = S.oprow + (size_t)((b0 / S.tl_K) % S.nlist) * GF2_OUTER_LISTS;
	u64 *Tm = S.Tm + (size_t)((b0 / S.tl_K) % S.nlist) * ((size_t)GF2_KMAX * GF2_KMAX * GF2_GMAX * 64 * GF2_GMAX);
	k_outer_prow<<<dim3(1, S.nsys), dim3(256), 0, st>>>(b0 * G, b1 - b0, S.panels, S.aux, gprow, S.ss());
	if (!S.kn.outer_chain)
		k_outer_trsm<4, true><<<dim3((unsigned)(npan / 4), S.nsys), dim3(256), 0, st>>>(S.M, S.rows, S.srows, b0 * G, npan, 0, S.panels, S.aux, S.mult,
		                                                                               set_words, b0 % S.nsets, S.nsets, S.impl->T, Tm, S.ss());
	HIPCHK(hipGetLastError());
	return GF2BV_OK;
}

int enqueue_outer_apply(Solver &S, hipStream_t st, int b0, int b1, i64 t_begin, i64 t_end)
{
	const int G = S.impl->G;
	const i64 nt = t_end - t_begin;
	if (nt <= 0) return GF2BV_OK;
	const i64 set_words = (i64)G * mult_rows(S.rows);
	int *gprow = S.oprow + (size_t)((b0 / S.tl_K) % S.nlist) * GF2_OUTER_LISTS;
	const int npan = (b1 - b0) * G;
	if (S.kn.outer_chain) {
		const i64 g_begin = t_begin * TW / 4, ng = t_end * TW / 4 - g_begin;
		k_outer_trsm<4, false><<<dim3((unsigned)ng, S.nsys), dim3(256), 0, st>>>(S.M, S.rows, S.srows, b0 * G, npan, (int)g_begin, S.panels, S.aux,
		                                                                          S.mult, set_words, b0 % S.nsets, S.nsets, S.impl->T, (u64 *)nullptr, S.ss());
	} else
		k_outer_apply<<<dim3((unsigned)nt, S.nsys), dim3(512), 0, st>>>(S.M, S.rows, S.srows, b1 - b0, (const int *)gprow,
		                                                                (const u64 *)(S.Tm + (size_t)((b0 / S.tl_K) % S.nlist) * ((size_t)GF2_KMAX * GF2_KMAX * GF2_GMAX * 64 * GF2_GMAX)), (int)t_begin, S.ss());
	HIPCHK(hipGetLastError());
	hipEvent_t ka = nullptr, kb = nullptr;
	if (S.time_kernels) {
		HIPCHK(pool().event(&ka, true)); HIPCHK(pool().event(&kb, true));
		S.kev.push_back(ka); S.kev.push_back(kb);
	}
	const i64 est_lo = std::min<i64>(S.rows, (i64)b0 * 64 * G) & ~(i64)63, R64 = round_up(S.rows, 64);
	constexpr i64 item_rows = (i64)GF2_WSEG * 1024;
	static_assert((size_t)item_rows * 32 <= kOuterSlackBytes, "the slack behind the matrix covers an item");
	const i64 nch = std::max<i64>(1, (R64 - est_lo + item_rows - 1) / item_rows);
	const i64 wgs = std::min<i64>(nch * nt, (i64)1 << 30);
	hipExtLaunchKernelGGL(k_update16k_wide, dim3((unsigned)wgs, S.nsys), dim3(1024), 0, st, ka, kb, 0,
	                      S.M, S.rows, S.srows, b1 - b0, (const int *)gprow, (const u64 *)S.mult,
	                      set_words, b0 % S.nsets, S.nsets, (const int *)(S.blk_first + b0), (const int *)S.died, b1 * G, (int)t_begin, (int)nt, S.ss(), 1);
	HIPCHK(hipGetLastError());
	if (S.kn.debug_sync & 2) HIPCHK(hipDeviceSynchronize());
	return GF2BV_OK;
}

int enqueue_window_gather(Solver &S, int b)
{
	const BlockGeom g = block_geom(S, b);
	k_win_gather<<<dim3((unsigned)((S.rows * g.gb + 255) / 256), S.nsys), dim3(256), 0, S.sA>>>(S.M, S.rows, S.srows, g.j0, g.gb, S.Wb, S.st, S.ss());
	HIPCHK(hipGetLastError());
	return GF2BV_OK;
}

int enqueue_forward(Solver &S)
{
	Trace tr;
	int rc = enqueue_forward_begin(S, true);
	if (rc) return rc;
	bool optimistic = false;
	SolveState hst{};
	const bool may_probe = S.kn.fast && S.optimistic && S.nsys == 1 && S.world == 1 && S.nblocks >= 8 && fast_block_possible(S, block_geom(S, 0));
	auto fast_only_ok = [&](int blk) {
		return fast_block_possible(S, block_geom(S, blk)) && S.rows - (i64)blk * 64 * S.impl->G >= GF2_FAST_NC + 128;
	};
	const bool may_sparse = may_probe && S.kn.sparse_fast && S.tl_K == 0;
	int general_only = -1;
	auto sparse_ok = [&](int blk) { return S.sparse_on && blk != general_only && fast_block_possible(S, block_geom(S, blk)); };
	auto recover = [&](int pb) -> int {
		if (S.sC) HIPCHK(hipStreamSynchronize(S.sC));
		HIPCHK(hipStreamSynchronize(S.sB));
		if (S.tl_K && pb < S.tl_bend) S.tl_bend = pb / S.tl_K * S.tl_K;
		S.bulk_waits_outer = false;
		HIPCHK(hipMemsetAsync(&S.st->poison, 0, sizeof(int), S.sA));
		S.sync_base += S.nblocks + 1;
		return GF2BV_OK;
	};
	int sparse_probes = 1;
	auto one_block = [&](int blk) -> int {
		int r;
		bool sp = sparse_ok(blk);
		if ((r = enqueue_block_panel(S, blk, sp || (optimistic && fast_only_ok(blk)), sp))) return r;
		if (sp && sparse_probes > 0) {
			sparse_probes--;
			HIPCHK(hipMemcpyAsync(&hst, S.st, sizeof hst, hipMemcpyDeviceToHost, S.sA));
			HIPCHK(hipStreamSynchronize(S.sA));
			const int want = hst.sp_nz > 3400 ? 2 : 0;
			if (hst.poison) {
				if ((r = recover(blk))) return r;
				if (++S.sparse_giveups >= 3) S.sparse_on = false; else sparse_probes = 1;
				S.sparse_tier = std::min(2, std::max(S.sparse_tier + 1, want));
				general_only = blk;
				if ((r = enqueue_block_panel(S, blk, false, false))) return r;
			} else S.sparse_tier = std::max(S.sparse_tier, want);
		}
		if ((r = enqueue_block_bulk(S, blk))) return r;
		if ((r = enqueue_block_prio(S, blk))) return r;
		if (blk == 0 && may_probe) {
			HIPCHK(hipMemcpyAsync(&hst, S.st, sizeof hst, hipMemcpyDeviceToHost, S.sA));
			HIPCHK(hipStreamSynchronize(S.sA));
			optimistic = hst.fast_done == 1;
			if (!optimistic && may_sparse && S.nblocks > 1) {
				S.sparse_on = true;
				const BlockGeom g1 = block_geom(S, 1);
				k_window_masks<<<dim3((unsigned)((S.rows + 255) / 256), S.nsys), dim3(256), 0, S.sA>>>((const u64 *)S.Wb, S.rows, g1.gb, (const int *)S.died, S.wmask,
				                                                                                      (const SolveState *)S.st, S.ss());
				HIPCHK(hipGetLastError());
			}
		}
		return GF2BV_OK;
	};
	int b = 0;
	if (S.tl_K) {
		const int G = S.impl->G;
		hipStream_t so = S.sC ? S.sC : S.sB;
		bool big_recorded = false;
		for (int p0 = 0; p0 < S.tl_bend; p0 += S.tl_K) {
			const int p1 = p0 + S.tl_K;
			if (p0 > 0) {
				HIPCHK(hipStreamWaitEvent(S.sA, S.evPri, 0));
				if ((rc = enqueue_window_gather(S, p0))) return rc;
			}
			S.tile_hi = (i64)p1 * G / TW;
			for (b = p0; b < p1; b++)
				if ((rc = one_block(b))) return rc;
			S.tile_hi = S.ntiles;
			if ((rc = enqueue_outer_prepare(S, S.sA, p0, p1))) return rc;
			HIPCHK(hipEventRecord(S.evPanelDone, S.sA));
			HIPCHK(hipStreamWaitEvent(so, S.evPanelDone, 0));
			const i64 t_out = S.ntiles;
			const i64 t0 = (i64)p1 * G / TW, t1 = std::min<i64>(t_out, t0 + (i64)S.tl_K * G / TW);
			const bool side = S.kn.outer_side && S.sB != so && S.sB != S.sA;
			if (side) {
				HIPCHK(hipStreamWaitEvent(S.sB, S.evPanelDone, 0));
				if (big_recorded) HIPCHK(hipStreamWaitEvent(S.sB, S.evBig, 0));
				if ((rc = enqueue_outer_apply(S, S.sB, p0, p1, t0, t1))) return rc;
				HIPCHK(hipEventRecord(S.evPri, S.sB));
				if ((rc = enqueue_outer_apply(S, so, p0, p1, t1, t_out))) return rc;
			} else {
				if ((rc = enqueue_outer_apply(S, so, p0, p1, t0, t1))) return rc;
				HIPCHK(hipEventRecord(S.evPri, so));
				if ((rc = enqueue_outer_apply(S, so, p0, p1, t1, t_out))) return rc;
			}
			HIPCHK(hipEventRecord(S.evBig, so));
			big_recorded = true;
		}
		HIPCHK(hipEventRecord(S.evOuter, so));
		b = S.tl_bend;
		HIPCHK(hipStreamWaitEvent(S.sA, S.evPri, 0));
		if (b < S.nblocks && (rc = enqueue_window_gather(S, b))) return rc;
		S.bulk_waits_outer = S.sC != nullptr;
	}
	for (; b < S.nblocks; b++)
		if ((rc = one_block(b))) return rc;
	if ((rc = enqueue_forward_join(S))) return rc;
	tr.mark(S.kn, "forward: all blocks submitted");
	while (optimistic || S.sparse_on) {
		HIPCHK(hipMemcpyAsync(&hst, S.st, sizeof hst, hipMemcpyDeviceToHost, S.sA));
		HIPCHK(hipStreamSynchronize(S.sA));
		if (!hst.poison) break;
		{
			const int pb = hst.poison - 1;
			if ((rc = recover(pb))) return rc;
			optimistic = false;
			if (S.sparse_on && ++S.sparse_giveups > 3) S.sparse_on = false;
			S.sparse_tier = std::min(2, S.sparse_tier + 1);
			general_only = pb;
			for (b = pb; b < S.nblocks; b++)
				if ((rc = one_block(b))) return rc;
			if ((rc = enqueue_forward_join(S))) return rc;
		}
	}
	return enqueue_check_rhs(S);
}

int enqueue_backward(Solver &S, const std::vector<int> &ycols_host)
{
	S.ny = (int)ycols_host.size();
	const i64 nyw = (S.ny + 63) / 64;
	S.ys = round_up(nyw, YTW);
	HIPCHK(pool().alloc((void **)&S.ycols, sizeof(int) * S.ny, S.device));
	HIPCHK(hipMemcpyAsync(S.ycols, ycols_host.data(), sizeof(int) * S.ny, hipMemcpyHostToDevice, S.sA));
	HIPCHK(pool().alloc((void **)&S.Y, sizeof(u64) * std::max<i64>(1, S.maxr) * S.ys, S.device));
	HIPCHK(hipMemsetAsync(S.Y, 0, sizeof(u64) * std::max<i64>(1, S.maxr) * S.ys, S.sA));
	HIPCHK(pool().alloc((void **)&S.out, sizeof(u64) * S.ny * std::max<i64>(1, S.cw), S.device));
	HIPCHK(hipMemsetAsync(S.out, 0, sizeof(u64) * S.ny * std::max<i64>(1, S.cw), S.sA));
	u64 *bmult = S.mult;
	const int rpb = 2048;
	if (S.maxr > 0) {
		const i64 kchunk = std::max<i64>(1, (1ll << 24) / nyw);
		for (i64 k0 = 0; k0 < S.maxr; k0 += kchunk) {
			const i64 waves = std::min(kchunk, S.maxr - k0) * nyw;
			k_extract_y<<<dim3((unsigned)((waves + 3) / 4)), dim3(256), 0, S.sA>>>(S.M, S.srows, S.st, S.urow, S.pivcol,
			                                                                      S.ycols, S.ny, S.Y, S.ys, k0);
		}
		const int ytiles = (int)(S.ys / YTW);
		for (int q = S.npanels - 1; q >= 1; q--) {
			const i64 bound = std::min<i64>((i64)64 * q, S.maxr);
			int g = (int)std::min<i64>(1024, (bound + 255) / 256);
			k_gather_mult_u<<<dim3(g), dim3(256), 0, S.sA>>>(S.M, S.srows, q, S.panels + q, S.urow, bmult);
			const i64 nrb = (bound + rpb - 1) / rpb;
			HIPCHK(launch_ysweep(dim3((unsigned)(ytiles * nrb)), S.sA, S.Y, S.ys, S.maxr, S.panels + q, bmult, ytiles, rpb));
		}
		for (i64 k0 = 0; k0 < S.maxr; k0 += kchunk << 6) {
			const i64 thr = std::min(kchunk << 6, S.maxr - k0) * nyw;
			k_scatter_solution<<<dim3((unsigned)((thr + 255) / 256)), dim3(256), 0, S.sA>>>(S.Y, S.ys, S.st, S.pivcol, S.ny,
			                                                                              S.out, std::max<i64>(1, S.cw), k0);
		}
	}
	HIPCHK(hipGetLastError());
	HIPCHK(hipEventRecord(S.ev2, S.sA));
	return GF2BV_OK;
}

int enqueue_backward_parity(Solver &S, const std::vector<int> &ycols_host)
{
	S.ny = (int)ycols_host.size();
	const i64 cw = std::max<i64>(1, S.cw);
	HIPCHK(pool().alloc((void **)&S.ycols, sizeof(int) * S.ny, S.device));
	HIPCHK(hipMemcpyAsync(S.ycols, ycols_host.data(), sizeof(int) * S.ny, hipMemcpyHostToDevice, S.sA));
	HIPCHK(pool().alloc((void **)&S.out, sizeof(u64) * S.ny * cw, S.device));
	HIPCHK(hipMemsetAsync(S.out, 0, sizeof(u64) * S.ny * cw, S.sA));
	unsigned char *accv = reinterpret_cast<unsigned char *>(S.mult);
	const i64 nacc = std::max<i64>(1, S.maxr);
	HIPCHK(pool().alloc((void **)&S.Y, sizeof(u64) * 64 * 16 * std::max(1, S.npanels), S.device));
	if (S.npanels > 0)
		k_bs_diag<<<dim3(S.npanels), dim3(256), 0, S.sA>>>(S.M, S.srows, S.npanels, S.panels, S.urow, S.Y, SysStride{0, 0}, (i64)0);
	const int ngroups = (S.npanels + GF2_BSG - 1) / GF2_BSG;
	const bool inv = S.kn.bs_inv >= 0 ? S.kn.bs_inv != 0 && ngroups >= 1 : ngroups >= 16;
	if (inv) {
		HIPCHK(pool().alloc((void **)&S.Minv, sizeof(u64) * (size_t)ngroups * 16 * 64 * 16, S.device));
		static std::mutex mu;
		static std::map<int, bool> raised;
		{
			std::lock_guard<std::mutex> lk(mu);
			if (!raised[S.device]) {
				HIPCHK(hipFuncSetAttribute((const void *)k_bs_inv, hipFuncAttributeMaxDynamicSharedMemorySize, GF2_BSINV_LDS));
				raised[S.device] = true;
			}
		}
		k_bs_inv<<<dim3(ngroups), dim3(1024), GF2_BSINV_LDS, S.sA>>>(S.Y, S.npanels, S.panels, S.pivcol, S.Minv);
	}
	for (int v0 = 0; v0 < S.ny; v0 += GF2_BSV) {
		const int nv = std::min(GF2_BSV, S.ny - v0);
		for (int qb = S.npanels; qb > 0; qb -= GF2_BSG) {
			const int qa = std::max(0, qb - GF2_BSG);
			const int waves = (qb - qa) * 64;
			k_bs_far<<<dim3((waves + 3) / 4), dim3(256), 0, S.sA>>>(S.M, S.srows, cw, qa, qb, S.panels, S.urow, S.pivcol, S.ycols + v0, nv,
			                                                        S.out + (i64)v0 * cw, accv, nacc, SysStride{0, 0}, (i64)0);
			if (inv)
				k_bs_near2<<<dim3(1), dim3(1024), 0, S.sA>>>(cw, qa, qb, S.panels, S.pivcol, nv, S.out + (i64)v0 * cw, accv, nacc, S.Minv,
				                                             (S.npanels - qb) / GF2_BSG);
			else
				k_bs_near<<<dim3(1), dim3(256), 0, S.sA>>>(S.Y, cw, qa, qb, S.panels, S.pivcol, nv, S.out + (i64)v0 * cw, accv, nacc,
				                                           SysStride{0, 0}, (i64)0, (i64)0);
		}
	}
	HIPCHK(hipGetLastError());
	HIPCHK(hipEventRecord(S.ev2, S.sA));
	return GF2BV_OK;
}

int enqueue_backward_gang(Solver &S)
{
	S.ny = 1;
	const i64 cw = std::max<i64>(1, S.cw);
	S.h_ycol = (int)S.cols;
	HIPCHK(pool().alloc((void **)&S.ycols, sizeof(int), S.device));
	HIPCHK(hipMemcpyAsync(S.ycols, &S.h_ycol, sizeof(int), hipMemcpyHostToDevice, S.sA));
	HIPCHK(pool().alloc((void **)&S.out, sizeof(u64) * cw * S.nsys, S.device));
	HIPCHK(hipMemsetAsync(S.out, 0, sizeof(u64) * cw * S.nsys, S.sA));
	unsigned char *accv = reinterpret_cast<unsigned char *>(S.mult);
	const i64 nacc = std::max<i64>(1, S.maxr);
	const i64 dgw = (i64)64 * 16 * std::max(1, S.npanels);
	HIPCHK(pool().alloc((void **)&S.Y, sizeof(u64) * dgw * S.nsys, S.device));
	if (S.npanels > 0)
		k_bs_diag<<<dim3(S.npanels, S.nsys), dim3(256), 0, S.sA>>>(S.M, S.srows, S.npanels, S.panels, S.urow, S.Y, S.ss(), dgw);
	for (int qb = S.npanels; qb > 0; qb -= GF2_BSG) {
		const int qa = std::max(0, qb - GF2_BSG);
		const int waves = (qb - qa) * 64;
		k_bs_far<<<dim3((waves + 3) / 4, S.nsys), dim3(256), 0, S.sA>>>(S.M, S.srows, cw, qa, qb, S.panels, S.urow, S.pivcol, S.ycols, 1,
		                                                                S.out, accv, nacc, S.ss(), cw);
		k_bs_near<<<dim3(1, S.nsys), dim3(256), 0, S.sA>>>(S.Y, cw, qa, qb, S.panels, S.pivcol, 1, S.out, accv, nacc, S.ss(), dgw, cw);
	}
	HIPCHK(hipGetLastError());
	HIPCHK(hipEventRecord(S.ev2, S.sA));
	return GF2BV_OK;
}

int enqueue_backsub(Solver &S, const std::vector<int> &ycols)
{
	if ((i64)ycols.size() <= GF2_BS_MAXRHS && !S.kn.ysweep) return enqueue_backward_parity(S, ycols);
	return enqueue_backward(S, ycols);
}

int solver_enqueue(Solver &S)
{
	Trace tr;
	int rc = solver_alloc(S);
	tr.mark(S.kn, "solver_alloc");
	if (rc) return rc;
	rc = enqueue_forward(S);
	tr.mark(S.kn, "enqueue_forward");
	if (rc) return rc;
	if (S.mode == GF2BV_MODE_SINGLE) return enqueue_backsub(S, { (int)S.cols });
	return GF2BV_OK;
}

std::vector<int> m4ri_free_order(const int32_t *piv, i64 rank, i64 cols)
{
	std::vector<int> order(cols);
	for (i64 i = 0; i < cols; i++) order[i] = (int)i;
	for (i64 i = 0; i < rank; i++) std::swap(order[i], order[piv[i]]);
	return std::vector<int>(order.begin() + rank, order.end());
}

int load_free_order(Solver &S)
{
	HIPCHK(hipMemcpyAsync(&S.hst, S.st, sizeof S.hst, hipMemcpyDeviceToHost, S.sA));
	HIPCHK(hipStreamSynchronize(S.sA));
	std::vector<int32_t> piv(S.hst.rank);
	if (S.hst.rank)
		HIPCHK(hipMemcpy(piv.data(), S.pivcol, sizeof(int) * S.hst.rank, hipMemcpyDeviceToHost));
	S.free_order = m4ri_free_order(piv.data(), S.hst.rank, S.cols);
	return GF2BV_OK;
}

int enqueue_export(Solver &S)
{
	HIPCHK(pool().event(&S.evx, true));
	HIPCHK(hipMemcpyAsync(&S.hst, S.st, sizeof S.hst, hipMemcpyDeviceToHost, S.sA));
	S.hout.resize((size_t)S.ny * std::max<i64>(1, S.cw));
	HIPCHK(hipMemcpyAsync(S.hout.data(), S.out, sizeof(u64) * S.hout.size(), hipMemcpyDeviceToHost, S.sA));
	S.hp.resize(std::max(1, S.npanels));
	HIPCHK(hipMemcpyAsync(S.hp.data(), S.panels, sizeof(PanelRec) * S.hp.size(), hipMemcpyDeviceToHost, S.sA));
	S.hpiv.resize(std::max<i64>(1, S.maxr));
	HIPCHK(hipMemcpyAsync(S.hpiv.data(), S.pivcol, sizeof(int) * S.hpiv.size(), hipMemcpyDeviceToHost, S.sA));
	HIPCHK(hipEventRecord(S.evx, S.sA));
	return GF2BV_OK;
}

int finish_begin(Solver &S)
{
	if (S.mode == GF2BV_MODE_AFFINE_SPACE) {
		int rc = load_free_order(S);
		if (rc) return rc;
		std::vector<int> yc;
		if (!S.hst.inconsistent) yc = S.free_order;
		yc.push_back((int)S.cols);
		if ((rc = enqueue_backsub(S, yc))) return rc;
	}
	return enqueue_export(S);
}

int handover_verdict(Solver &S)
{
	if (!S.hst.gate_timeout) return GF2BV_OK;
	if (!S.flag_sync) return fail(GF2BV_ERR_HIP, "a stream hand-over gate timed out on the device");
	forget_concurrency(S.device);
	return GF2BV_RETRY_EVENTS;
}

std::unique_ptr<gf2bv_result> new_result(bool solved, i64 cols, const int32_t *piv, i64 rank, const u64 *origin)
{
	const i64 cw = (cols + 63) / 64;
	std::unique_ptr<gf2bv_result> R(new gf2bv_result());
	R->status = solved ? GF2BV_STATUS_SOLVED : GF2BV_STATUS_INCONSISTENT;
	R->rank = rank;
	R->cw = cw;
	R->dim = cols - rank;
	R->pivots.assign(piv, piv + rank);
	R->origin.assign((size_t)std::max<i64>(1, cw), 0);
	if (solved) std::copy(origin, origin + cw, R->origin.begin());
	return R;
}

std::vector<u64> basis_rows(const u64 *hout, i64 cw, const std::vector<int> &free_order, i64 dim)
{
	const i64 cwx = std::max<i64>(1, cw);
	std::vector<u64> basis((size_t)(dim * cwx), 0);
	for (i64 t = 0; t < dim; t++) {
		u64 *v = basis.data() + (size_t)(t * cwx);
		std::copy(hout + (size_t)(t * cwx), hout + (size_t)(t * cwx + cw), v);
		const int f = free_order[(size_t)t];
		v[f >> 6] |= 1ull << (f & 63);
	}
	return basis;
}

void fill_stats(const Solver &S, gf2bv_result *R);

int finish_end(Solver &S, gf2bv_result **out)
{
	Trace tr;
	HIPCHK(hipStreamSynchronize(S.sA));
	HIPCHK(hipStreamSynchronize(S.sB));
	tr.mark(S.kn, "finish: sync");
	int rc = handover_verdict(S);
	if (rc) return rc;
	const SolveState &hst = S.hst;
	const i64 cwx = std::max<i64>(1, S.cw);
	S.hpiv.resize(hst.rank);
	std::unique_ptr<gf2bv_result> R = new_result(!hst.inconsistent, S.cols, S.hpiv.data(), hst.rank, S.hout.data() + (size_t)((S.ny - 1) * cwx));
	if (!hst.inconsistent && S.mode == GF2BV_MODE_AFFINE_SPACE) R->basis = basis_rows(S.hout.data(), S.cw, S.free_order, R->dim);
	fill_stats(S, R.get());
	tr.mark(S.kn, "finish: result");
	*out = R.release();
	return GF2BV_OK;
}

void fill_stats(const Solver &S, gf2bv_result *R)
{
	const SolveState &hst = S.hst;
	const std::vector<PanelRec> &hp = S.hp;
	const hipEvent_t evx = S.evx;
	gf2bv_stats &st = R->stats;
	st.rows = S.rows; st.cols = S.cols; st.stride_words = S.stride;
	st.rank = R->rank; st.dimension = R->dim; st.status = R->status;
	st.n_panels = S.npanels;
	st.panels_per_sweep = S.impl->G;
	st.tables_per_sweep = S.impl->G * S.impl->T;
	st.table_bits = (64 + S.impl->T - 1) / S.impl->T;
	st.tile_words = TW;
	st.gang_systems = S.view ? S.gang_nsys : S.nsys;
	st.search_handovers = hst.self_giveups;
	st.fast_blocks = hst.fast_blocks;
	{
		const int G = S.impl->G;
		for (int b = 0; b < S.nblocks; b++) {
			const int j0 = b * G, gb = std::min(G, S.npanels - j0), wlo = j0 + gb;
			int pend = 0, any = 0;
			for (int g = 0; g < gb; g++) { any |= hp[j0 + g].p; pend = hp[j0 + g].start + hp[j0 + g].p; }
			if (!any || wlo >= S.wt) continue;
			const double rows_swept = (double)(S.rows - pend);
			st.n_sweeps++;
			st.sweep_words += rows_swept * (double)(S.wt - wlo);
			st.row_xors += rows_swept * (double)(S.impl->T * gb);
			if (S.tl_K && b < S.tl_bend) {
				const int pend_w = (b / S.tl_K + 1) * S.tl_K * G;
				const i64 out_w = S.wt;
				st.outer_blocks++;
				if (pend_w > wlo) { st.hbm_words += rows_swept * (double)(std::min<i64>(pend_w, S.wt) - wlo); st.bulk_launches++; }
				if ((b + 1) % S.tl_K == 0 && out_w > pend_w) { st.hbm_words += rows_swept * (double)(out_w - pend_w); st.bulk_launches += 2; }
			} else { st.hbm_words += rows_swept * (double)(S.wt - wlo); st.bulk_launches++; }
		}
	}
	st.ms_pack = S.ms_pack;
	st.handover_retries = g_attempt;
	(void)hipEventElapsedTime(&st.ms_eliminate, S.ev0, S.ev1);
	(void)hipEventElapsedTime(&st.ms_backsub, S.ev1, S.ev2);
	(void)hipEventElapsedTime(&st.ms_export, S.ev2, evx);
// ... 1579 lines not shown
	rc = solver_finish(S, out);
	if (rc == GF2BV_RETRY_EVENTS) return fail(GF2BV_ERR_HIP, "a stream hand-over gate timed out on the device");
	return rc;
	});
}

void gf2bv_slab_close(gf2bv_slab *h)
{
	if (!h) return;
	(void)hipSetDevice(h->S.device);
	delete h;
}

struct gf2bv_space {
	int device = 0;
	int64_t dim = 0, words = 0;
	u64 *d_origin = nullptr, *d_basis = nullptr;
	u64 *d_out = nullptr;
	u64 *h_out = nullptr;
	size_t out_words = 0;
	hipStream_t st = nullptr;
};

int gf2bv_space_open(const uint64_t *origin, const uint64_t *basis, int64_t dimension, int64_t words, int device,
                     gf2bv_space **out)
{
	return guarded([&]() -> int {
	if (!out || !origin || dimension < 0 || words <= 0 || (dimension > 0 && !basis)) return fail(GF2BV_ERR_ARG, "bad space");
	*out = nullptr;
	int rc = check_device(device);
	if (rc) return rc;
	gf2bv_space *sp = new gf2bv_space();
	sp->device = device; sp->dim = dimension; sp->words = words;
	auto bail = [&](hipError_t e, const char *what) { gf2bv_space_close(sp); return fail(GF2BV_ERR_HIP, what, e); };
	hipError_t e = pool().stream(&sp->st, device, false);
	if (e != hipSuccess) return bail(e, "hipStreamCreate");
	if ((e = pool().alloc((void **)&sp->d_origin, sizeof(u64) * words, device)) != hipSuccess) return bail(e, "hipMalloc");
	if ((e = pool().alloc((void **)&sp->d_basis, sizeof(u64) * std::max<i64>(1, dimension * words), device)) != hipSuccess) return bail(e, "hipMalloc");
	if ((e = hipMemcpyAsync(sp->d_origin, origin, sizeof(u64) * words, hipMemcpyHostToDevice, sp->st)) != hipSuccess) return bail(e, "hipMemcpy");
	if (dimension > 0 && (e = hipMemcpyAsync(sp->d_basis, basis, sizeof(u64) * dimension * words, hipMemcpyHostToDevice, sp->st)) != hipSuccess)
		return bail(e, "hipMemcpy");
	if ((e = hipStreamSynchronize(sp->st)) != hipSuccess) return bail(e, "hipStreamSynchronize");
	*out = sp;
	return GF2BV_OK;
	});
}

int gf2bv_space_enumerate(gf2bv_space *sp, uint64_t first, int64_t count, int gray, uint64_t *out_words)
{
	return guarded([&]() -> int {
	if (!sp || count < 0) return fail(GF2BV_ERR_ARG, "null pointer");
	if (count == 0) return GF2BV_OK;
	HIPCHK(hipSetDevice(sp->device));
	const size_t need = (size_t)count * sp->words;
	if (need > sp->out_words) {
		pool().release(sp->d_out); sp->d_out = nullptr; sp->out_words = 0;
		if (sp->h_out) { (void)hipHostFree(sp->h_out); sp->h_out = nullptr; }
		HIPCHK(pool().alloc((void **)&sp->d_out, sizeof(u64) * need, sp->device));
		HIPCHK(hipHostMalloc((void **)&sp->h_out, sizeof(u64) * need, hipHostMallocDefault));
		sp->out_words = need;
	}
	const dim3 grid((unsigned)((sp->words + 255) / 256), (unsigned)std::min<i64>(count, 65535));
	k_space_enumerate<<<grid, dim3(256), 0, sp->st>>>(sp->d_origin, sp->d_basis, (int)std::min<i64>(sp->dim, 64), sp->words,
	                                                  (u64)first, (i64)count, gray, sp->d_out);
	HIPCHK(hipGetLastError());
	HIPCHK(hipMemcpyAsync(sp->h_out, sp->d_out, sizeof(u64) * need, hipMemcpyDeviceToHost, sp->st));
	HIPCHK(hipStreamSynchronize(sp->st));
	if (out_words) memcpy(out_words, sp->h_out, sizeof(u64) * need);
	return GF2BV_OK;
	});
}

const uint64_t *gf2bv_space_buffer(const gf2bv_space *sp) { return sp ? reinterpret_cast<const uint64_t *>(sp->h_out) : nullptr; }

void gf2bv_space_close(gf2bv_space *sp)
{
	if (!sp) return;
	(void)hipSetDevice(sp->device);
	if (sp->st) (void)hipStreamSynchronize(sp->st);
	pool().release(sp->d_origin); pool().release(sp->d_basis); pool().release(sp->d_out);
	if (sp->h_out) (void)hipHostFree(sp->h_out);
	if (sp->st) pool().release_stream(sp->st, sp->device, false);
	delete sp;
}

int gf2bv_synth_device(void *d_aug, int64_t rows, int64_t cols, int64_t stride_words, uint64_t seed,
                       int device, void *stream)
{
	if (!d_aug || rows < 0 || cols <= 0 || stride_words < (cols + 1 + 63) / 64 || rows >= (1ll << 20) - 1)
		return fail(GF2BV_ERR_ARG, "bad synthetic shape");
	int rc = check_device(device);
	if (rc) return rc;
	if (rows == 0) return GF2BV_OK;
	hipLaunchKernelGGL(k_synth, dim3((unsigned)((rows + 3) / 4)), dim3(256), 0, (hipStream_t)stream,
	                   (u64 *)d_aug, (i64)rows, (i64)cols, (i64)stride_words, (u64)seed);
	HIPCHK(hipGetLastError());
	return GF2BV_OK;
}

int gf2bv_residual_device(const void *d_aug, int64_t rows, int64_t cols, int64_t stride_words,
                          const uint64_t *x_words, int device, void *stream, int64_t *bad_rows)
{
	if (!d_aug || !x_words || !bad_rows || cols <= 0) return fail(GF2BV_ERR_ARG, "null pointer");
	int rc = check_device(device);
	if (rc) return rc;
	const i64 cw = (cols + 63) / 64;
	u64 *dx = nullptr, *dbad = nullptr;
	HIPCHK(hipMalloc(&dx, sizeof(u64) * cw));
	HIPCHK(hipMalloc(&dbad, sizeof(u64)));
	hipStream_t s = (hipStream_t)stream;
	HIPCHK(hipMemcpyAsync(dx, x_words, sizeof(u64) * cw, hipMemcpyHostToDevice, s));
	HIPCHK(hipMemsetAsync(dbad, 0, sizeof(u64), s));
	if (rows > 0)
		hipLaunchKernelGGL(k_residual, dim3((unsigned)((rows + 3) / 4)), dim3(256), 0, s,
		                   (const u64 *)d_aug, (i64)rows, (i64)cols, (i64)stride_words, dx, dbad);
	u64 h = 0;
	HIPCHK(hipMemcpyAsync(&h, dbad, sizeof h, hipMemcpyDeviceToHost, s));
	HIPCHK(hipStreamSynchronize(s));
	(void)hipFree(dx); (void)hipFree(dbad);
	*bad_rows = (int64_t)h;
	return GF2BV_OK;
}

int gf2bv_kernel_resources(int device, int32_t *out, int n)
{
	return guarded([&]() -> int {
	if (!out || n < 10) return fail(GF2BV_ERR_ARG, "need room for 5 kernels");
	for (int k = 0; k < n; k++) out[k] = 0;
	int rc = check_device(device);
	if (rc) return rc;
	HIPCHK(hipSetDevice(device));
	const void *fn[5] = { (const void *)k_update16<512, false, 3, true, 512>, (const void *)k_block_fast, (const void *)k_narrow_all,
	                      (const void *)k_prio_window, (const void *)k_panel_step };
	for (int k = 0; k < 5; k++) {
		hipFuncAttributes a{};
		HIPCHK(hipFuncGetAttributes(&a, fn[k]));
		out[2 * k] = a.numRegs;
		out[2 * k + 1] = (int32_t)a.sharedSizeBytes;
	}
	if (n >= 13) {
		hipFuncAttributes a{};
		HIPCHK(hipFuncGetAttributes(&a, (const void *)k_update16k_wide));
		out[10] = a.numRegs; out[11] = (int32_t)a.sharedSizeBytes; out[12] = (int32_t)a.localSizeBytes;
	}
	if (n >= 15) {
		hipFuncAttributes a{};
		HIPCHK(hipFuncGetAttributes(&a, (const void *)k_block_fast_narrow));
		out[13] = a.numRegs; out[14] = (int32_t)a.sharedSizeBytes;
	}
	if (n >= 17) {
		hipFuncAttributes a{};
		HIPCHK(hipFuncGetAttributes(&a, (const void *)k_block_sparse<256, 4>));
		out[15] = a.numRegs; out[16] = (int32_t)a.sharedSizeBytes;
	}
	return GF2BV_OK;
	});
}

int gf2bv_stream_ceiling_device(int device, int64_t bytes, double *rmw_gbs, double *read_gbs)
{
	if (!rmw_gbs || !read_gbs || bytes < (1 << 20)) return fail(GF2BV_ERR_ARG, "bad ceiling request");
	int rc = check_device(device);
	if (rc) return rc;
	const int wgs = 2048;
	const i64 per = bytes / 16 / wgs;
	uint4 *buf = nullptr;
	unsigned *sink = nullptr;
	hipError_t e = hipMalloc(&buf, (size_t)per * wgs * 16);
	if (e != hipSuccess) return fail(GF2BV_ERR_NOMEM, "hipMalloc", e);
	HIPCHK(hipMalloc(&sink, 64));
	HIPCHK(hipMemset(buf, 1, (size_t)per * wgs * 16));
	hipEvent_t e0, e1;
	HIPCHK(hipEventCreate(&e0)); HIPCHK(hipEventCreate(&e1));
	const int reps = 5;
	float ms = 0;
	k_rmw_stream<<<dim3(wgs), dim3(1024)>>>(buf, per, 5u);
	HIPCHK(hipEventRecord(e0, nullptr));
	for (int r = 0; r < reps; r++) k_rmw_stream<<<dim3(wgs), dim3(1024)>>>(buf, per, 5u);
	HIPCHK(hipEventRecord(e1, nullptr));
	HIPCHK(hipEventSynchronize(e1));
	HIPCHK(hipEventElapsedTime(&ms, e0, e1));
	*rmw_gbs = 2.0 * (double)per * wgs * 16 * reps / (ms * 1e-3) / 1e9;
	k_read_stream<<<dim3(wgs), dim3(1024)>>>(buf, per, sink);
	HIPCHK(hipEventRecord(e0, nullptr));
	for (int r = 0; r < reps; r++) k_read_stream<<<dim3(wgs), dim3(1024)>>>(buf, per, sink);
	HIPCHK(hipEventRecord(e1, nullptr));
	HIPCHK(hipEventSynchronize(e1));
	HIPCHK(hipEventElapsedTime(&ms, e0, e1));
	*read_gbs = (double)per * wgs * 16 * reps / (ms * 1e-3) / 1e9;
	(void)hipEventDestroy(e0); (void)hipEventDestroy(e1);
	(void)hipFree(buf); (void)hipFree(sink);
	return GF2BV_OK;
}

int gf2bv_lds_clock_device(int device, double *shader_mhz, double *lds_bytes_per_clk_cu)
{
	if (!shader_mhz || !lds_bytes_per_clk_cu) return fail(GF2BV_ERR_ARG, "null pointer");
	int rc = check_device(device);
	if (rc) return rc;
	unsigned long long *d = nullptr, h[3] = { 0, 0, 0 };
	unsigned *sink = nullptr;
	struct Free { unsigned long long *&d; unsigned *&sink; ~Free() { pool().release(d); pool().release(sink); } } guard{ d, sink };
	HIPCHK(pool().alloc((void **)&d, sizeof h, device));
	HIPCHK(pool().alloc((void **)&sink, 64, device));
	int cus = 256;
	(void)hipDeviceGetAttribute(&cus, hipDeviceAttributeMultiprocessorCount, device);
	k_lds_clock<<<dim3(cus), dim3(512)>>>(d, 2000, sink);
	k_lds_clock<<<dim3(cus), dim3(512)>>>(d, 40000, sink);
	HIPCHK(hipGetLastError());
	HIPCHK(hipMemcpy(h, d, sizeof h, hipMemcpyDeviceToHost));
	if (!h[1]) return fail(GF2BV_ERR_HIP, "the clock probe measured nothing");
	*shader_mhz = (double)h[0] / ((double)h[1] / 100.0);
	*lds_bytes_per_clk_cu = (double)h[2] * 1024.0 / (double)h[0];
	return GF2BV_OK;
}

int gf2bv_device_alloc(int device, int64_t bytes, void **d_ptr)
{
	if (!d_ptr || bytes < 0) return fail(GF2BV_ERR_ARG, "bad alloc request");
	int rc = check_device(device);
	if (rc) return rc;
	hipError_t e = pool().malloc_retry(d_ptr, (size_t)std::max<i64>(bytes, 16), device);
	if (e != hipSuccess) return fail(GF2BV_ERR_NOMEM, "hipMalloc", e);
	return GF2BV_OK;
}
namespace {
struct HostPool {
	std::mutex mu;
	struct Buf { void *p; size_t bytes; };
	std::vector<Buf> idle;
	std::unordered_map<void *, size_t> live;
};
HostPool *host_pool_ptr() { static HostPool *p = new HostPool(); return p; }
}
int gf2bv_host_alloc(int64_t bytes, void **h_ptr)
{
	if (!h_ptr || bytes < 0) return fail(GF2BV_ERR_ARG, "bad alloc request");
	*h_ptr = nullptr;
	const size_t need = std::max<size_t>((size_t)bytes, 64);
	HostPool &P = *host_pool_ptr();
	{
		std::lock_guard<std::mutex> lk(P.mu);
		for (size_t i = 0; i < P.idle.size(); i++)
			if (P.idle[i].bytes >= need && P.idle[i].bytes <= 2 * need + ((size_t)1 << 20)) {
				*h_ptr = P.idle[i].p; P.live[*h_ptr] = P.idle[i].bytes;
				P.idle.erase(P.idle.begin() + i);
				return GF2BV_OK;
			}
	}
	int n = 0;
	if (hipGetDeviceCount(&n) != hipSuccess || n <= 0) return fail(GF2BV_ERR_NODEVICE, "no HIP device visible");
	void *p = nullptr;
	const size_t cap = need + need / 8;
	hipError_t e = hipHostMalloc(&p, cap, hipHostMallocDefault);
	if (e != hipSuccess) { (void)hipGetLastError(); return fail(GF2BV_ERR_NOMEM, "hipHostMalloc", e); }
	std::lock_guard<std::mutex> lk(P.mu);
	P.live[p] = cap;
	*h_ptr = p;
	return GF2BV_OK;
}
void gf2bv_host_free(void *h_ptr)
{
	if (!h_ptr) return;
	HostPool &P = *host_pool_ptr();
	void *drop = nullptr;
	{
		std::lock_guard<std::mutex> lk(P.mu);
		auto it = P.live.find(h_ptr);
		if (it == P.live.end()) return;
		const size_t bytes = it->second;
		P.live.erase(it);
		size_t kept = 0;
		for (const auto &b : P.idle) kept += b.bytes;
		const size_t cap_mb = (size_t)Knobs::read(Knobs::kHostPool).host_pool_mb;
		if (P.idle.size() < 4 && kept + bytes <= (cap_mb << 20)) P.idle.push_back({ h_ptr, bytes });
		else drop = h_ptr;
	}
	if (drop) (void)hipHostFree(drop);
}

int64_t gf2bv_host_pool_trim(void)
{
	HostPool &P = *host_pool_ptr();
	std::vector<HostPool::Buf> drop;
	{
		std::lock_guard<std::mutex> lk(P.mu);
		drop.swap(P.idle);
	}
	int64_t bytes = 0;
	for (const auto &b : drop) { bytes += (int64_t)b.bytes; (void)hipHostFree(b.p); }
	return bytes;
}

int64_t gf2bv_plan_gang(int64_t nsys, int64_t rows, int64_t cols, int64_t free_bytes)
{
	if (nsys <= 0 || rows <= 0 || cols <= 0 || free_bytes < 0) return 0;
	return pick_gang(Knobs::read(), nsys, rows, cols, free_bytes);
}

int gf2bv_knob_dump(char *buf, int64_t n)
{
	return catching([&]() -> int {
	const std::string s = Knobs::read().dump();
	if (!buf || (int64_t)s.size() >= n) return fail(GF2BV_ERR_ARG, "null pointer, or a buffer too small for the knob dump");
	memcpy(buf, s.c_str(), s.size() + 1);
	return GF2BV_OK;
// ... 2320 lines not shown
```

gf2bv_amd/hip.py:

```python
from __future__ import annotations

import ctypes
import os
from dataclasses import dataclass, field

import numpy as np

_HERE = os.path.dirname(os.path.abspath(__file__))
LIB_PATH = os.environ.get("GF2BV_LIB") or os.path.join(_HERE, "libgf2bv_hip.so")

MODE_SINGLE = 0
MODE_AFFINE_SPACE = 1
STATUS_SOLVED = 0
STATUS_INCONSISTENT = 1

EXPORTS = [
    "gf2bv_version", "gf2bv_build_id", "gf2bv_device_count", "gf2bv_last_error",
    "gf2bv_solve_digits", "gf2bv_solve_words", "gf2bv_solve_device", "gf2bv_solve_batch_device",
    "gf2bv_solve_batch_digits", "gf2bv_solve_batch_digits_multi",
    "gf2bv_solve_rhs_digits", "gf2bv_solve_rhs_words", "gf2bv_solve_rhs_device",
    "gf2bv_factor_digits", "gf2bv_factor_words", "gf2bv_factor_device", "gf2bv_factor_solve", "gf2bv_factor_solve_device",
    "gf2bv_factor_rank", "gf2bv_factor_pivots", "gf2bv_factor_device_bytes", "gf2bv_factor_free",
    "gf2bv_factor_append_words", "gf2bv_factor_append_digits", "gf2bv_factor_append_device", "gf2bv_factor_rows",
    "gf2bv_factor_copy",
# ... 1009 lines not shown

def xl4_guess_chunk(m: int, n_lin: int, nguess: int, free_bytes: int | None = None, device: int = 0) -> int:
    return _xl_guess_chunk(4, m, n_lin, nguess, free_bytes, device)


def _cubic_rows(cubic) -> np.ndarray:
    cubic = np.ascontiguousarray(cubic, dtype=np.uint64)
    if cubic.ndim != 2:
        raise ValueError("the cubic rows must be a 2-D uint64 array, one row per equation")
    return cubic


def xl4_cubic_expand_words(cubic, n_lin: int, rows: int | None = None, stride_words: int | None = None, device: int = 0) -> np.ndarray:
    cubic = _cubic_rows(cubic)
    m = len(cubic)
    rows = m * (n_lin + 1) if rows is None else rows
    stride = (xl4_cols(n_lin) + 1 + 63) // 64 if stride_words is None else stride_words
    out = np.empty((max(rows, 0), max(stride, 0)), dtype=np.uint64)
    _check(lib().gf2bv_xl4_cubic_expand_words(cubic.ctypes.data, m, cubic.shape[1], n_lin, rows, out.ctypes.data, stride, device))
    return out


def xl4_cubic_expand_device(d_cubic: int, m: int, cubic_stride: int, n_lin: int, rows: int, d_aug: int, stride: int, device: int = 0,
                            stream: int = 0) -> None:
    _check(lib().gf2bv_xl4_cubic_expand_device(d_cubic, m, cubic_stride, n_lin, rows, d_aug, stride, device, stream or None))


def solve_xl4_cubic_words(cubic, n_lin: int, mode: int = MODE_SINGLE, device: int = 0) -> Solution:
    cubic = _cubic_rows(cubic)
    h = ctypes.c_void_p()
    _check(lib().gf2bv_solve_xl4_cubic_words(cubic.ctypes.data, len(cubic), cubic.shape[1], n_lin, mode, device, ctypes.byref(h)))
    return _take(h, mode)


def solve_xl4_cubic_terms(lin, off2, ta, tb, off3, ua, ub, uc, n_lin: int, mode: int = MODE_SINGLE, device: int = 0) -> Solution:
    terms = _terms(n_lin, lin, off2, ta, tb, off3, ua, ub, uc)
    h = ctypes.c_void_p()
    _check(lib().gf2bv_solve_xl4_cubic_terms(*_ptrs(*terms), len(terms[0]), n_lin, mode, device, ctypes.byref(h)))
    return _take(h, mode)


def cubic_specialise_words(cubic, n_lin: int, guess, a0: int = 0, na: int | None = None, stride_words: int | None = None,
                           device: int = 0) -> np.ndarray:
    cubic, guess = _cubic_rows(cubic), _guess(guess)
    na = _assignments(guess, a0, na)
    stride = (xl3_cols(n_lin - len(guess)) + 1 + 63) // 64 if stride_words is None else stride_words
    out = np.empty((max(na, 0), len(cubic), max(stride, 0)), dtype=np.uint64)
    _check(lib().gf2bv_cubic_specialise_words(cubic.ctypes.data, len(cubic), cubic.shape[1], n_lin, guess.ctypes.data, len(guess), a0, na,
                                              out.ctypes.data, stride, device))
    return out


def cubic_specialise_device(d_cubic: int, m: int, cubic_stride: int, n_lin: int, guess, a0: int, na: int, d_out: int, out_stride: int,
                            sys_stride: int, device: int = 0, stream: int = 0) -> None:
    guess = _guess(guess)
    _check(lib().gf2bv_cubic_specialise_device(d_cubic, m, cubic_stride, n_lin, guess.ctypes.data, len(guess), a0, na, d_out, out_stride,
                                               sys_stride, device, stream or None))


def xl4_cubic_expand_batch_words(cubics, n_lin: int, rows: int | None = None, stride_words: int | None = None,
                                 sys_stride_words: int | None = None, device: int = 0) -> np.ndarray:
    cubics = np.ascontiguousarray(cubics, dtype=np.uint64)
    if cubics.ndim != 3:
        raise ValueError("the systems must be a 3-D uint64 array: system, equation, word")
    nsys, m, cs = cubics.shape
    rows = m * (n_lin + 1) if rows is None else rows
    stride = (xl4_cols(n_lin) + 1 + 63) // 64 if stride_words is None else stride_words
    sys_stride = rows * stride if sys_stride_words is None else sys_stride_words
    out = np.zeros((nsys, max(sys_stride, 0)), dtype=np.uint64)
    _check(lib().gf2bv_xl4_cubic_expand_batch_words(cubics.ctypes.data, nsys, m * cs, m, cs, n_lin, rows, out.ctypes.data, stride, sys_stride,
                                                    device))
    return out


def xl4_cubic_expand_batch_device(d_cubic: int, nsys: int, cubic_sys_stride: int, m: int, cubic_stride: int, n_lin: int, rows: int, d_aug: int,
                                  stride: int, sys_stride: int, device: int = 0, stream: int = 0) -> None:
    _check(lib().gf2bv_xl4_cubic_expand_batch_device(d_cubic, nsys, cubic_sys_stride, m, cubic_stride, n_lin, rows, d_aug, stride, sys_stride,
                                                     device, stream or None))


def solve_xl4_cubic_guess_words(cubic, n_lin: int, guess, a0: int = 0, na: int | None = None, mode: int = MODE_SINGLE, device: int = 0) -> list:
    cubic, guess = _cubic_rows(cubic), _guess(guess)
    na = _assignments(guess, a0, na)
    hs = _handles(na)
    rc = lib().gf2bv_solve_xl4_cubic_guess_words(cubic.ctypes.data, len(cubic), cubic.shape[1], n_lin, guess.ctypes.data, len(guess), a0, na,
                                                 mode, device, hs)
    return _take_all(hs, max(na, 0), rc, mode)


def solve_xl4_cubic_guess_terms(lin, off2, ta, tb, off3, ua, ub, uc, n_lin: int, guess, a0: int = 0, na: int | None = None,
                                mode: int = MODE_SINGLE, device: int = 0) -> list:
    terms = _terms(n_lin, lin, off2, ta, tb, off3, ua, ub, uc)
    guess = _guess(guess)
    na = _assignments(guess, a0, na)
    hs = _handles(na)
    rc = lib().gf2bv_solve_xl4_cubic_guess_terms(*_ptrs(*terms), len(terms[0]), n_lin, guess.ctypes.data, len(guess), a0, na, mode, device, hs)
    return _take_all(hs, max(na, 0), rc, mode)


def xl4_cubic_guess_chunk(m: int, n_lin: int, nguess: int, free_bytes: int | None = None, device: int = 0) -> int:
    if free_bytes is None:
        chunk = ctypes.c_int64()
        _check(lib().gf2bv_xl4_cubic_guess_chunk_device(m, n_lin, nguess, device, ctypes.byref(chunk)))
        return int(chunk.value)
    chunk = int(lib().gf2bv_xl4_cubic_guess_chunk(m, n_lin, nguess, free_bytes))
    if chunk < 0:
        raise ValueError("m, n_lin, nguess or free_bytes out of range")
    return chunk


def synth_device(d_ptr: int, rows: int, cols: int, stride: int, seed: int, device: int = 0, stream: int = 0):
    _check(lib().gf2bv_synth_device(d_ptr, rows, cols, stride, seed, device, stream or None))


def _mix64(x: np.ndarray) -> np.ndarray:
    with np.errstate(over="ignore"):
        x = x + np.uint64(0x9E3779B97F4A7C15)
        x = (x ^ (x >> np.uint64(30))) * np.uint64(0xBF58476D1CE4E5B9)
        x = (x ^ (x >> np.uint64(27))) * np.uint64(0x94D049BB133111EB)
        return x ^ (x >> np.uint64(31))


def planted_solution(cols: int, seed: int) -> np.ndarray:
    cw = (cols + 63) // 64
    s = _mix64(np.array([seed], dtype=np.uint64))[0]
    x = _mix64(s ^ (np.uint64(0xFFFFF << 20) | np.arange(cw, dtype=np.uint64)))
    if cols & 63:
        x[-1] &= np.uint64((1 << (cols & 63)) - 1)
    return x


def residual_device(d_ptr: int, rows: int, cols: int, stride: int, x: np.ndarray, device: int = 0,
                    stream: int = 0) -> int:
    x = np.ascontiguousarray(x, dtype=np.uint64)
    bad = ctypes.c_int64(-1)
    _check(lib().gf2bv_residual_device(d_ptr, rows, cols, stride, x.ctypes.data, device, stream or None,
                                       ctypes.byref(bad)))
    return int(bad.value)


def stream_ceiling(nbytes: int = 2 << 30, device: int = 0) -> dict:
    rmw, rd = ctypes.c_double(0), ctypes.c_double(0)
    _check(lib().gf2bv_stream_ceiling_device(device, nbytes, ctypes.byref(rmw), ctypes.byref(rd)))
    return {"rmw_gbs": rmw.value, "read_gbs": rd.value}


def lds_clock(device: int = 0) -> dict:
    mhz, bpc = ctypes.c_double(0), ctypes.c_double(0)
    _check(lib().gf2bv_lds_clock_device(device, ctypes.byref(mhz), ctypes.byref(bpc)))
    return {"shader_mhz": mhz.value, "lds_bytes_per_clk_cu": bpc.value}


def kernel_resources(device: int = 0) -> dict:
    out = (ctypes.c_int32 * 20)()
    _check(lib().gf2bv_kernel_resources(device, out, 20))
    names = ("update", "block_fast", "narrow_all", "prio_window", "panel_step")
    res = {nm: {"vgprs": int(out[2 * k]), "lds": int(out[2 * k + 1])} for k, nm in enumerate(names)}
    res["update_outer"] = {"vgprs": int(out[10]), "lds": int(out[11]), "scratch": int(out[12])}
    res["block_fast_narrow"] = {"vgprs": int(out[13]), "lds": int(out[14])}
    res["block_sparse"] = {"vgprs": int(out[15]), "lds": int(out[16])}
    return res


def pool_trim(device: int = 0) -> int:
    return int(lib().gf2bv_pool_trim(device))


def knobs() -> dict:
    buf = ctypes.create_string_buffer(4096)
    _check(lib().gf2bv_knob_dump(buf, len(buf)))
    return dict(line.split("=", 1) for line in buf.value.decode().splitlines())


def host_pool_trim() -> int:
    return int(lib().gf2bv_host_pool_trim())


def pool_idle_bytes(device: int = 0) -> int:
    return int(lib().gf2bv_pool_idle_bytes(device))


class DeviceBuffer:

    def __init__(self, nbytes: int, device: int = 0):
        self.device, self.nbytes = device, nbytes
        p = ctypes.c_void_p()
        _check(lib().gf2bv_device_alloc(device, nbytes, ctypes.byref(p)))
        self.ptr = p.value

    def upload(self, arr: np.ndarray):
        arr = np.ascontiguousarray(arr)
        _check(lib().gf2bv_device_upload(self.device, self.ptr, arr.ctypes.data, arr.nbytes))

    def download(self, dtype=np.uint64) -> np.ndarray:
        out = np.zeros(self.nbytes // np.dtype(dtype).itemsize, dtype=dtype)
        _check(lib().gf2bv_device_download(self.device, out.ctypes.data, self.ptr, self.nbytes))
        return out

    def free(self):
        if self.ptr:
            lib().gf2bv_device_free(self.device, self.ptr)
            self.ptr = None

    def __del__(self):
        try:
            self.free()
        except Exception:
            pass


def padded_stride(cols: int, multiple: int = 32) -> int:
    wt = (cols + 1 + 63) // 64
    return (wt + multiple - 1) // multiple * multiple
```

Before: 8.118 billion.

## Update head rows first and launch next block's TRSM early on a side stream

The trailing update kernel gains a head-first variant that processes the leading rows of each tile first with write-through stores, then signals a head-done flag before finishing the rest. The next block's TRSM can then run on a third stream once the head is done, falling back to waiting on bulk completion if its source rows lie beyond the head region. This is meant to shorten the critical path between consecutive blocks by overlapping TRSM with the tail of the bulk update. It adds flags, gating kernels, stream dependencies, and a pinned-register kernel instance, which risks extra sync overhead, register spills, or stalls waiting on timeouts.

```diff
diff --git a/gf2bv_amd/csrc/gf2_kernels.hip.h b/gf2bv_amd/csrc/gf2_kernels.hip.h
--- a/gf2bv_amd/csrc/gf2_kernels.hip.h
+++ b/gf2bv_amd/csrc/gf2_kernels.hip.h
@@ -65,7 +65,11 @@
 	int narrow_done;
 	int bulk_done;
 	unsigned cnt_narrow;
+	int head_done;
+	int trsm_done;
+	unsigned cnt_head;
 };
+#define GF2_HEAD_ROWS ((64 + 8 * 256 + 511) / 512 * 512)
 struct DoneSignal { unsigned *count; int *flag; int value; };
 
 struct FindUnit {
@@ -278,15 +282,17 @@
 }
 __global__ void __launch_bounds__(64)
 k_gate(SyncFlags *__restrict__ sf, SolveState *__restrict__ st, int set_narrow, int set_bulk, int need_narrow, int need_bulk,
-       SysStride ss)
+       SysStride ss, int set_trsm, int need_trsm, int need_head)
 {
 	sf = sys_at(sf, blockIdx.y * ss.arena_bytes); st = sys_at(st, blockIdx.y * ss.arena_bytes);
 	if (threadIdx.x != 0) return;
 	if (set_narrow > 0) GF2_ST(&sf->narrow_done, set_narrow);
 	if (set_bulk > 0) GF2_ST(&sf->bulk_done, set_bulk);
+	if (set_trsm > 0) GF2_ST(&sf->trsm_done, set_trsm);
 	const unsigned long long t0 = wall_clock64();
 	int polls = 0;
-	while (GF2_LD(&sf->narrow_done) < need_narrow || GF2_LD(&sf->bulk_done) < need_bulk) {
+	while (GF2_LD(&sf->narrow_done) < need_narrow || GF2_LD(&sf->bulk_done) < need_bulk ||
+	       (need_trsm > 0 && GF2_LD(&sf->trsm_done) < need_trsm) || (need_head > 0 && GF2_LD(&sf->head_done) < need_head)) {
 		if (++polls < 512) __builtin_amdgcn_s_sleep(2); else __builtin_amdgcn_s_sleep(64);
 		if (wall_clock64() - t0 > GF2_GATE_TICKS || GF2_LD(&st->gate_timeout)) { GF2_ST(&st->gate_timeout, 1); break; }
 	}
@@ -1955,17 +1961,18 @@
 }
 
 
-template <int TW, int WPW>
+template <int TW, int WPW, bool EARLY = false>
 __global__ void __launch_bounds__(64 * WPW)
 k_block_trsm(u64 *__restrict__ M, i64 srows, int j0, int gb, int wlo, int group_begin, int world, int wrank,
              const PanelRec *__restrict__ panels, const PanelAux *__restrict__ aux, int nw_lo, int nw_hi, u64 *__restrict__ Pc,
-             SysStride ss)
+             SysStride ss, SyncFlags *__restrict__ sf, SolveState *__restrict__ st, const int *__restrict__ prev_first, int need_bulk)
 {
 	__builtin_amdgcn_s_setprio(2);
 	M += blockIdx.y * ss.m_words;
 	panels = sys_at(panels, blockIdx.y * ss.arena_bytes);
 	aux = sys_at(aux, blockIdx.y * ss.arena_bytes);
 	if (Pc) Pc = sys_at(Pc, blockIdx.y * ss.arena_bytes);
+	if (EARLY) { sf = sys_at(sf, blockIdx.y * ss.arena_bytes); st = sys_at(st, blockIdx.y * ss.arena_bytes); prev_first = sys_at(prev_first, blockIdx.y * ss.arena_bytes); }
 	constexpr int NT = 64 * WPW;
 	static_assert(WPW == 4 && NT == 256, "thread <-> table entry mapping below");
 	__shared__ u64 S[GF2_GMAX * 64 * WPW];
@@ -1990,9 +1997,26 @@
 		for (int e = 0; e < GF2_GMAX; e++) smul[g][e] = (e < g) ? aux[j0 + gc].src_mult[r][e] : 0ull;
 		if (g >= gb) { rec[g].p = 0; rec[g].mask = 0; }
 	}
+	if (EARLY) {
+		const i64 hend = ((i64)(*prev_first) & ~(i64)63) + GF2_HEAD_ROWS;
+		int ok = GF2_LD(&st->poison) == 0;
+#pragma unroll
+		for (int g = 0; g < GF2_GMAX; g++) if (r < rec[g].p && srow[g] >= hend) ok = 0;
+		if (!__syncthreads_and(ok)) {
+			if (t == 0) {
+				const unsigned long long t0 = wall_clock64();
+				while (GF2_LD(&sf->bulk_done) < need_bulk) {
+					__builtin_amdgcn_s_sleep(8);
+					if (wall_clock64() - t0 > GF2_GATE_TICKS || GF2_LD(&st->gate_timeout)) { GF2_ST(&st->gate_timeout, 1); break; }
+				}
+			}
+			__syncthreads();
+		}
+	}
 #pragma unroll
 	for (int g = 0; g < GF2_GMAX; g++) {
-		const u64 v = at(r < rec[g].p ? srow[g] : 0);
+		u64 *const src = &at(r < rec[g].p ? srow[g] : 0);
+		const u64 v = EARLY ? GF2_LD(src) : *src;
 		S[(g * 64 + r) * WPW + w] = (r < rec[g].p && live) ? v : 0ull;
 		Pbit[(g * 64 + r) * WPW + w] = 0;
 		if (w == 0 && ((rec[g].mask >> r) & 1)) Bk[g * 64 + __popcll(rec[g].mask & lanemask_lt(r))] = r;
@@ -2063,13 +2087,15 @@
 typedef unsigned u32x4 __attribute__((ext_vector_type(4)));
 typedef __attribute__((address_space(3))) const u32x4 *lds_u4_ptr;
 
-template <int NT, bool HALF, int DEPTH, bool PIPE, int LB, bool STREAM = false>
-__global__ void __launch_bounds__(LB)
-k_update16(u64 *__restrict__ M, i64 rows, i64 srows, int j0, int gb, int wlo,
-           const PanelRec *__restrict__ panels, const PanelAux *__restrict__ aux,
-           const u64 *__restrict__ mult4, const int *__restrict__ blk_first,
-           int tile_begin, int ntiles, int world, int wrank, const uint4 *__restrict__ Pc, SysStride ss, int xcd_nsys)
-{
+template <bool B> struct BoolC { static constexpr bool value = B; };
+#define GF2_U16_PARAMS u64 *__restrict__ M, i64 rows, i64 srows, int j0, int gb, int wlo, \
+	const PanelRec *__restrict__ panels, const PanelAux *__restrict__ aux, const u64 *__restrict__ mult4, const int *__restrict__ blk_first, \
+	int tile_begin, int ntiles, int world, int wrank, const uint4 *__restrict__ Pc, SysStride ss, int xcd_nsys, DoneSignal head
+#define GF2_U16_ARGS M, rows, srows, j0, gb, wlo, panels, aux, mult4, blk_first, tile_begin, ntiles, world, wrank, Pc, ss, xcd_nsys, head
+template <int NT, bool HALF, int DEPTH, bool PIPE, bool STREAM, bool HEADF>
+__device__ __forceinline__ void update16_body(GF2_U16_PARAMS)
+{
+	static_assert(!HEADF || (!HALF && !STREAM), "head-first order: the plain full-tile instance only");
 	unsigned bx = blockIdx.x, gx = gridDim.x, by = blockIdx.y;
 	if (xcd_nsys > 0) {
 		const unsigned slot = bx >> 3, xcd = bx & 7;
@@ -2092,7 +2118,10 @@
 
 	int anyp = 0;
 	for (int g = 0; g < gb; g++) anyp |= panels[j0 + g].p;
-	if (!anyp) return;
+	if (!anyp) {
+		if (HEADF) signal_light(head, (i64)by * ss.arena_bytes, gx);
+		return;
+	}
 	const i64 rlo = (i64)(*blk_first) & ~(i64)63;
 	const i64 R64 = (rows + 63) & ~(i64)63;
 	constexpr int ALIGN = NW * 64;
@@ -2121,11 +2150,43 @@
 
 	unsigned sgx = 0, sgy = 0, sgz = 0, sgw = 0;
 	bool have_staged = false;
-	for (bool first_span = true; pos < pend; first_span = false) {
-		const int ct = (int)(pos / R);
-		const i64 r0 = pos - (i64)ct * R;
-		const i64 span = (R - r0 < pend - pos) ? R - r0 : pend - pos;
-		pos += span;
+	constexpr i64 HEAD = GF2_HEAD_ROWS;
+	static_assert(!HEADF || HEAD % ALIGN == 0, "the heads end on a step of the streaming loop");
+	const i64 pos0 = pos;
+	const int c_first = R > 0 ? (int)(pos0 / R) : 0;
+	const int npieces = (HEADF && pos0 < pend) ? (int)((pend - 1) / R) - c_first + 1 : 0;
+	auto item_rows = [&](int j, int &ct, i64 &a, i64 &e) {
+		const bool rest = j >= npieces;
+		const int jj = rest ? j - npieces : j;
+		const int i = rest ? (jj == 0 ? npieces - 1 : jj - 1) : jj;
+		ct = c_first + i;
+		const i64 s = i == 0 ? pos0 - (i64)c_first * R : 0, t = i == npieces - 1 ? pend - (i64)ct * R : R;
+		a = rest ? (s > HEAD ? s : HEAD) : s;
+		e = rest ? t : (t < HEAD ? t : HEAD);
+		return a < e && rlo + a < R64;
+	};
+	int item = 0, cur_ct = -1, staged_ct = -1;
+	for (bool first_span = true; HEADF || pos < pend; first_span = false) {
+		int ct;
+		i64 r0, span;
+		bool wthru = false, build = true;
+		if (HEADF) {
+			if (item == npieces) signal_light(head, (i64)by * ss.arena_bytes, gx);
+			if (item >= 2 * npieces) break;
+			i64 a, e;
+			const bool any = item_rows(item, ct, a, e);
+			wthru = item < npieces;
+			item++;
+			if (!any) continue;
+			r0 = a; span = e - a;
+			build = ct != cur_ct;
+			cur_ct = ct;
+		} else {
+			ct = (int)(pos / R);
+			r0 = pos - (i64)ct * R;
+			span = (R - r0 < pend - pos) ? R - r0 : pend - pos;
+			pos += span;
+		}
 		const i64 tile = owned_item(ct, tile_begin, GF2_OWN_LOG - 1, world, wrank);
 		const i64 rbeg = rlo + r0;
 		if (rbeg >= R64) continue;
@@ -2155,65 +2216,76 @@
 #pragma unroll
 			for (int d = 0; d < DEPTH - 1; d++) load(H[d], d);
 		}
-		if (!first_span) __syncthreads();
-		if (first_span && !Pc) {
-			for (int t = threadIdx.x; t < GF2_GMAX * 64; t += NT) {
-				const int g = t >> 6, b = t & 63;
-				int pr = -1;
-				if (g < gb) {
-					const PanelRec rec = panels[j0 + g];
-					if ((rec.mask >> b) & 1) pr = aux[j0 + g].slot_row[__popcll(rec.mask & ((1ull << b) - 1))];
+		if (build) {
+			if (!first_span) __syncthreads();
+			if (first_span && !Pc) {
+				for (int t = threadIdx.x; t < GF2_GMAX * 64; t += NT) {
+					const int g = t >> 6, b = t & 63;
+					int pr = -1;
+					if (g < gb) {
+						const PanelRec rec = panels[j0 + g];
+						if ((rec.mask >> b) & 1) pr = aux[j0 + g].slot_row[__popcll(rec.mask & ((1ull << b) - 1))];
+					}
+					prow[t] = pr;
 				}
-				prow[t] = pr;
+				__syncthreads();
+			}
+			const uint4 *Mq = reinterpret_cast<const uint4 *>(M) + tile * srows;
+			if (threadIdx.x < GF2_GMAX * 64) {
+				const int pr = Pc ? 0 : prow[threadIdx.x];
+				uint4 v;
+				if (have_staged && (!HEADF || staged_ct == ct)) { v.x = sgx; v.y = sgy; v.z = sgz; v.w = sgw; }
+				else v = Pc ? Pc[tile * (GF2_GMAX * 64) + threadIdx.x] : Mq[pr >= 0 ? pr : 0];
+				const bool k0 = pr >= 0 && 2 * tile >= wlo, k1 = pr >= 0 && 2 * tile + 1 >= wlo;
+				if (!k0) { v.x = 0; v.y = 0; }
+				if (!k1) { v.z = 0; v.w = 0; }
+				stage[threadIdx.x] = v;
 			}
 			__syncthreads();
-		}
-		const uint4 *Mq = reinterpret_cast<const uint4 *>(M) + tile * srows;
-		if (threadIdx.x < GF2_GMAX * 64) {
-			const int pr = Pc ? 0 : prow[threadIdx.x];
-			uint4 v;
-			if (have_staged) { v.x = sgx; v.y = sgy; v.z = sgz; v.w = sgw; }
-			else v = Pc ? Pc[tile * (GF2_GMAX * 64) + threadIdx.x] : Mq[pr >= 0 ? pr : 0];
-			const bool k0 = pr >= 0 && 2 * tile >= wlo, k1 = pr >= 0 && 2 * tile + 1 >= wlo;
-			if (!k0) { v.x = 0; v.y = 0; }
-			if (!k1) { v.z = 0; v.w = 0; }
-			stage[threadIdx.x] = v;
-		}
-		__syncthreads();
-		for (int it = threadIdx.x; it < 2 * 31 * 16; it += NT) {
-			const int sub = it & 15, e = (it >> 4) % 31, grp = (it >> 4) / 31;
-			const int idx = e <= 15 ? e : (e - 15) << 4;
-			const uint4 *st = stage + (2 * grp + (sub >> 3)) * 64 + 8 * (sub & 7);
-			uint4 acc = make_uint4(0, 0, 0, 0);
-			int bits = idx;
-			while (bits) {
-				const int l = __ffs(bits) - 1; bits &= bits - 1;
-				acc = xor4(acc, st[l]);
-			}
-			tab[grp * 4096 + idx * 16 + sub] = acc;
-		}
-		__syncthreads();
-		for (int it = threadIdx.x; it < 2 * 225 * 16; it += NT) {
-			const int sub = it & 15, k = (it >> 4) % 225, grp = (it >> 4) / 225;
-			const int lo = 1 + k % 15, hi = (1 + k / 15) << 4;
-			uint4 *tb = tab + grp * 4096 + sub;
-			tb[(lo | hi) * 16] = xor4(tb[lo * 16], tb[hi * 16]);
-		}
-		__syncthreads();
-
-		have_staged = false;
-		if (pos < pend) {
-			const i64 ntile = owned_item((int)(pos / R), tile_begin, GF2_OWN_LOG - 1, world, wrank);
-			if (threadIdx.x < GF2_GMAX * 64) {
-				uint4 nx;
-				if (Pc) nx = Pc[ntile * (GF2_GMAX * 64) + threadIdx.x];
-				else {
-					const int pr = prow[threadIdx.x];
-					nx = (reinterpret_cast<const uint4 *>(M) + ntile * srows)[pr >= 0 ? pr : 0];
+			for (int it = threadIdx.x; it < 2 * 31 * 16; it += NT) {
+				const int sub = it & 15, e = (it >> 4) % 31, grp = (it >> 4) / 31;
+				const int idx = e <= 15 ? e : (e - 15) << 4;
+				const uint4 *st = stage + (2 * grp + (sub >> 3)) * 64 + 8 * (sub & 7);
+				uint4 acc = make_uint4(0, 0, 0, 0);
+				int bits = idx;
+				while (bits) {
+					const int l = __ffs(bits) - 1; bits &= bits - 1;
+					acc = xor4(acc, st[l]);
 				}
-				sgx = nx.x; sgy = nx.y; sgz = nx.z; sgw = nx.w;
-			}
-			have_staged = true;
+				tab[grp * 4096 + idx * 16 + sub] = acc;
+			}
+			__syncthreads();
+			for (int it = threadIdx.x; it < 2 * 225 * 16; it += NT) {
+				const int sub = it & 15, k = (it >> 4) % 225, grp = (it >> 4) / 225;
+				const int lo = 1 + k % 15, hi = (1 + k / 15) << 4;
+				uint4 *tb = tab + grp * 4096 + sub;
+				tb[(lo | hi) * 16] = xor4(tb[lo * 16], tb[hi * 16]);
+			}
+			__syncthreads();
+
+			have_staged = false;
+			int nct = -1;
+			if (HEADF) {
+				for (int j = item; j < 2 * npieces && nct < 0; j++) {
+					int c;
+					i64 a, e;
+					if (item_rows(j, c, a, e) && c != ct) nct = c;
+				}
+			} else if (pos < pend) nct = (int)(pos / R);
+			if (nct >= 0) {
+				const i64 ntile = owned_item(nct, tile_begin, GF2_OWN_LOG - 1, world, wrank);
+				staged_ct = nct;
+				if (threadIdx.x < GF2_GMAX * 64) {
+					uint4 nx;
+					if (Pc) nx = Pc[ntile * (GF2_GMAX * 64) + threadIdx.x];
+					else {
+						const int pr = prow[threadIdx.x];
+						nx = (reinterpret_cast<const uint4 *>(M) + ntile * srows)[pr >= 0 ? pr : 0];
+					}
+					sgx = nx.x; sgy = nx.y; sgz = nx.z; sgw = nx.w;
+				}
+				have_staged = true;
+			}
 		}
 		auto issue = [&](u32x4 *v, const Bt &H, int r) {
 			const unsigned mw[8] = { H.m0.x, H.m0.y, H.m0.z, H.m0.w, H.m1.x, H.m1.y, H.m1.z, H.m1.w };
@@ -2235,13 +2307,17 @@
 				acc.w = __builtin_amdgcn_bitop3_b32(acc.w, v[2 * h].w, v[2 * h + 1].w, 0x96);
 			}
 		};
-		auto store = [&](const Bt &H, const uint4 &acc) {
+		auto store = [&](auto wt, const Bt &H, const uint4 &acc) {
 #ifdef GF2_MB_L2
 			const i64 q = H.row & 4095;
 #else
 			const i64 q = H.row;
 #endif
-			if (HALF) reinterpret_cast<u64 *>(Mw + q)[1] = ((u64)acc.w << 32) | acc.z;
+			if (decltype(wt)::value) {
+				u64 *const o = reinterpret_cast<u64 *>(Mw + q);
+				GF2_ST(o, ((u64)acc.y << 32) | acc.x); GF2_ST(o + 1, ((u64)acc.w << 32) | acc.z);
+			}
+			else if (HALF) reinterpret_cast<u64 *>(Mw + q)[1] = ((u64)acc.w << 32) | acc.z;
 #ifdef GF2_NT_STORE
 			else { const u32x4 t = { acc.x, acc.y, acc.z, acc.w }; __builtin_nontemporal_store(t, reinterpret_cast<u32x4 *>(Mw + q)); }
 #else
@@ -2249,37 +2325,45 @@
 			else Mw[q] = acc;
 #endif
 		};
-		if (nb > 0) {
-			u32x4 va[8], vb[8];
+		auto stream = [&](auto wt) {
+			if (nb > 0) {
+				u32x4 va[8], vb[8];
 #ifndef GF2_MB_NOLOOKUP
-			if (PIPE) issue(va, H[0], 0);
+				if (PIPE) issue(va, H[0], 0);
 #endif
-			for (i64 i = 0; i < nb; i += DEPTH) {
-#pragma unroll
-				for (int d = 0; d < DEPTH; d++) {
-					if (i + d >= nb) break;
-					load(H[(d + DEPTH - 1) % DEPTH], i + d + DEPTH - 1);
-					Bt &C = H[d];
-					uint4 acc = C.d;
+				for (i64 i = 0; i < nb; i += DEPTH) {
+#pragma unroll
+					for (int d = 0; d < DEPTH; d++) {
+						if (i + d >= nb) break;
+						load(H[(d + DEPTH - 1) % DEPTH], i + d + DEPTH - 1);
+						Bt &C = H[d];
+						uint4 acc = C.d;
 #ifdef GF2_MB_NOLOOKUP
-					acc.x ^= C.m0.x ^ C.m0.y ^ C.m0.z ^ C.m0.w; acc.y ^= C.m1.x ^ C.m1.y ^ C.m1.z ^ C.m1.w;
+						acc.x ^= C.m0.x ^ C.m0.y ^ C.m0.z ^ C.m0.w; acc.y ^= C.m1.x ^ C.m1.y ^ C.m1.z ^ C.m1.w;
 #else
-					if (PIPE) {
-						issue(vb, C, 1); fold(acc, va);
-						issue(va, C, 2); fold(acc, vb);
-						issue(vb, C, 3); fold(acc, va);
-						issue(va, H[(d + 1) % DEPTH], 0); fold(acc, vb);
-					} else {
-#pragma unroll
-						for (int r = 0; r < 4; r++) { issue(va, C, r); fold(acc, va); }
+						if (PIPE) {
+							issue(vb, C, 1); fold(acc, va);
+							issue(va, C, 2); fold(acc, vb);
+							issue(vb, C, 3); fold(acc, va);
+							issue(va, H[(d + 1) % DEPTH], 0); fold(acc, vb);
+						} else {
+#pragma unroll
+							for (int r = 0; r < 4; r++) { issue(va, C, r); fold(acc, va); }
+						}
+#endif
+						store(wt, C, acc);
 					}
-#endif
-					store(C, acc);
 				}
 			}
-		}
-	}
-}
+		};
+		if (HEADF && wthru) stream(BoolC<true>{}); else stream(BoolC<false>{});
+	}
+}
+template <int NT, bool HALF, int DEPTH, bool PIPE, int LB, bool STREAM = false>
+__global__ void __launch_bounds__(LB)
+k_update16(GF2_U16_PARAMS) { update16_body<NT, HALF, DEPTH, PIPE, STREAM, false>(GF2_U16_ARGS); }
+__global__ void __launch_bounds__(512) __attribute__((amdgpu_num_vgpr(92)))
+k_update16_head_first(GF2_U16_PARAMS) { update16_body<512, false, 3, true, false, true>(GF2_U16_ARGS); }
 
 
 #ifndef GF2_KMAX
diff --git a/gf2bv_amd/csrc/gf2_solver.hip b/gf2bv_amd/csrc/gf2_solver.hip
--- a/gf2bv_amd/csrc/gf2_solver.hip
+++ b/gf2bv_amd/csrc/gf2_solver.hip
@@ -445,33 +445,40 @@
 struct UpdateImpl {
 	int G, T, lds_bytes, threads;
 	hipError_t (*update)(dim3, hipStream_t, u64 *, i64, i64, int, int, int, const PanelRec *, const PanelAux *,
-	                     const u64 *, const int *, int, int, int, int, int, bool, const uint4 *, SysStride, hipEvent_t, hipEvent_t, int);
+	                     const u64 *, const int *, int, int, int, int, int, bool, const uint4 *, SysStride, hipEvent_t, hipEvent_t, int, DoneSignal);
 };
 
+constexpr bool update_has_head_first(int update) { return update == 0; }
 template <int NT, int DEPTH, bool PIPE, int LB>
 hipError_t launch_update16(dim3 grid, hipStream_t s, u64 *M, i64 rows, i64 srows, int j0, int gb, int wlo,
                            const PanelRec *panels, const PanelAux *aux, const u64 *multset, const int *blk_first,
                            int tile_begin, int ntiles, int world, int wrank, int nw_lo, bool stream_rows, const uint4 *Pc, SysStride ss,
-                           hipEvent_t begun, hipEvent_t done, int xcd_nsys)
+                           hipEvent_t begun, hipEvent_t done, int xcd_nsys, DoneSignal head)
 {
 	if (xcd_nsys > 0) grid = dim3(grid.x * grid.y);
+	if (head.count) {
+		if (!(NT == 512 && DEPTH == 3 && PIPE && LB == 512) || nw_lo < 0 || stream_rows || xcd_nsys > 0 || !Pc) return hipErrorInvalidValue;
+		hipExtLaunchKernelGGL(k_update16_head_first, grid, dim3(512), 0, s, begun, done, 0, M, rows, srows, j0, gb, wlo,
+		                      panels, aux, multset, blk_first, tile_begin, ntiles, world, wrank, Pc, ss, xcd_nsys, head);
+		return hipGetLastError();
+	}
 	{
 		if (stream_rows && NT == 512 && DEPTH == 3 && PIPE && LB == 512) {
 			if (nw_lo < 0)
 				hipExtLaunchKernelGGL((k_update16<512, true, 3, true, 512, true>), grid, dim3(512), 0, s, begun, done, 0, M, rows, srows, j0, gb, wlo,
-				                      panels, aux, multset, blk_first, tile_begin, ntiles, world, wrank, Pc, ss, xcd_nsys);
+				                      panels, aux, multset, blk_first, tile_begin, ntiles, world, wrank, Pc, ss, xcd_nsys, DoneSignal{});
 			else
 				hipExtLaunchKernelGGL((k_update16<512, false, 3, true, 512, true>), grid, dim3(512), 0, s, begun, done, 0, M, rows, srows, j0, gb, wlo,
-				                      panels, aux, multset, blk_first, tile_begin, ntiles, world, wrank, Pc, ss, xcd_nsys);
+				                      panels, aux, multset, blk_first, tile_begin, ntiles, world, wrank, Pc, ss, xcd_nsys, DoneSignal{});
 			return hipGetLastError();
 		}
 	}
 	if (nw_lo < 0)
 		hipExtLaunchKernelGGL((k_update16<NT, true, DEPTH, PIPE, LB>), grid, dim3(NT), 0, s, begun, done, 0, M, rows, srows, j0, gb, wlo,
-		                      panels, aux, multset, blk_first, tile_begin, ntiles, world, wrank, Pc, ss, xcd_nsys);
+		                      panels, aux, multset, blk_first, tile_begin, ntiles, world, wrank, Pc, ss, xcd_nsys, DoneSignal{});
 	else
 		hipExtLaunchKernelGGL((k_update16<NT, false, DEPTH, PIPE, LB>), grid, dim3(NT), 0, s, begun, done, 0, M, rows, srows, j0, gb, wlo,
-		                      panels, aux, multset, blk_first, tile_begin, ntiles, world, wrank, Pc, ss, xcd_nsys);
+		                      panels, aux, multset, blk_first, tile_begin, ntiles, world, wrank, Pc, ss, xcd_nsys, DoneSignal{});
 	return hipGetLastError();
 }
 #define UPDATE16_IMPL(NT, D, P, LB) { 4, 8, 2 * 256 * 256 + GF2_GMAX * 64 * 20, NT, launch_update16<NT, D, P, LB> }
@@ -546,6 +553,8 @@
 	bool optimistic = true;
 	bool xcd_pin = true;
 	int sync_base = 0;
+	bool may_early = false, early = false;
+	int head_pass = -1;
 	int units = 0;
 	bool sparse_on = false;
 	int sparse_giveups = 0;
@@ -567,6 +576,7 @@
 	float ms_pack = 0;
 };
 
+inline size_t pc_words(const SolverPlan &P) { return (size_t)2 * GF2_GMAX * 64 * (size_t)P.ntiles; }
 ArenaLayout arena_layout(const SolverPlan &P)
 {
 	const i64 R = std::max<i64>(1, P.rows), NP = std::max(1, P.npanels);
@@ -581,7 +591,7 @@
 	L.Wb = carve(sizeof(u64) * 2 * GF2_GMAX * R); L.Uwin = carve(sizeof(u64) * GF2_GMAX * (P.maxr + 64));
 	L.Pfast = carve(sizeof(u64) * GF2_GMAX * GF2_GMAX * 64); L.oprow = carve(sizeof(int) * GF2_OUTER_LISTS * P.nlist);
 	L.Tm = carve(P.tl_K ? P.nlist * sizeof(u64) * GF2_KMAX * GF2_KMAX * GF2_GMAX * 64 * GF2_GMAX : 0);
-	L.Pc = carve(P.kn.pc ? sizeof(u64) * 2 * GF2_GMAX * 64 * (size_t)P.ntiles : 0);
+	L.Pc = carve(P.kn.pc ? sizeof(u64) * pc_words(P) * (P.early ? 2 : 1) : 0);
 	L.wmask = carve(sizeof(u64) * 2 * (size_t)((R + 63) / 64 + 1));
 	L.stride = off;
 	return L;
@@ -789,6 +799,10 @@
 		if (rc) return rc;
 		S.flag_sync = ok != 0;
 	}
+	S.early = S.may_early && S.flag_sync && kn.flag_sync != 3 && S.nsys == 1 && S.world == 1 && !S.ext_M && S.tl_K == 0 && S.sB != S.sA &&
+	          kn.pc && kn.fast && kn.fused_narrow && S.optimistic && update_has_head_first(kn.update) && S.nblocks >= 8 && S.nrhs == 1;
+	S.head_pass = -1;
+	if (S.early) HIPCHK(pool().low_stream_for(kn, S.sA, S.device, &S.sC));
 	{
 		const ArenaLayout &L = S.lay = arena_layout(S);
 		S.sync_base = 0;
@@ -805,6 +819,7 @@
 	HIPCHK(pool().event(&S.ev1, true));
 	HIPCHK(pool().event(&S.ev2, true));
 	HIPCHK(pool().event(&S.ev3, true));
+	if (S.early) HIPCHK(pool().event(&S.evPri, false));
 	if (S.tl_K) {
 		for (hipEvent_t *e : { &S.evOuter, &S.evPri, &S.evPanelDone }) HIPCHK(pool().event(e, false));
 		if (S.sB != S.sA) { if (S.nsys == 1) HIPCHK(pool().low_stream_for(kn, S.sA, S.device, &S.sC)); else HIPCHK(pool().stream(&S.sC, S.device, 3)); }
@@ -895,20 +910,28 @@
 	return n;
 }
 
-int launch_trsm(Solver &S, hipStream_t st, int j0, int gb, int wlo, int nw_lo, int nw_hi)
+u64 *pc_of(const Solver &S, int b) { return S.Pc && S.early ? S.Pc + (size_t)(b & 1) * pc_words(S) : S.Pc; }
+
+int launch_trsm(Solver &S, hipStream_t st, int b, int j0, int gb, int wlo, int nw_lo, int nw_hi, bool early = false)
 {
 	constexpr int WPW = 4;
 	const i64 g0 = wlo / WPW, g1 = S.tile_hi * TW / WPW;
 	const i64 ng = owned_count(g0, g1, GF2_OWN_LOG - 2, S.world, S.wrank);
 	if (ng <= 0) return GF2BV_OK;
-	k_block_trsm<TW, WPW><<<dim3((unsigned)ng, S.nsys), dim3(64 * WPW), 0, st>>>(S.M, S.srows, j0, gb, wlo, (int)g0, S.world, S.wrank,
-	                                                                           S.panels, S.aux, nw_lo, nw_hi, S.Pc, S.ss());
+	if (early)
+		k_block_trsm<TW, WPW, true><<<dim3((unsigned)ng, S.nsys), dim3(64 * WPW), 0, st>>>(S.M, S.srows, j0, gb, wlo, (int)g0, S.world, S.wrank,
+		                                                                                 S.panels, S.aux, nw_lo, nw_hi, pc_of(S, b), S.ss(), S.sf, S.st,
+		                                                                                 (const int *)(S.blk_first + b - 1), S.sync_base + b);
+	else
+		k_block_trsm<TW, WPW><<<dim3((unsigned)ng, S.nsys), dim3(64 * WPW), 0, st>>>(S.M, S.srows, j0, gb, wlo, (int)g0, S.world, S.wrank,
+		                                                                           S.panels, S.aux, nw_lo, nw_hi, pc_of(S, b), S.ss(), (SyncFlags *)nullptr,
+		                                                                           (SolveState *)nullptr, (const int *)nullptr, 0);
 	HIPCHK(hipGetLastError());
 	return GF2BV_OK;
 }
 
 int launch_update_timed(Solver &S, hipStream_t st, int b, int j0, int gb, int wlo, u64 *mset, int tile_begin, int ntiles,
-                        int nw_lo, bool last, hipEvent_t *handoff)
+                        int nw_lo, bool last, hipEvent_t *handoff, bool head_first = false)
 {
 	hipEvent_t ka = nullptr, kb = nullptr;
 	if (S.time_kernels) {
@@ -921,7 +944,8 @@
 	const hipEvent_t begun = ka, done = S.time_kernels ? kb : (last && !S.flag_sync ? S.evPrio[b] : nullptr);
 	HIPCHK(S.impl->update(dim3((unsigned)wgs, S.nsys), st, S.M, S.rows, S.srows, j0, gb, wlo, S.panels, S.aux, mset,
 	                      S.blk_first + b, tile_begin, ntiles, S.world, S.wrank, nw_lo, pin && S.kn.gang_nt,
-	                      (const uint4 *)S.Pc, S.ss(), begun, done, pin ? S.nsys : 0));
+	                      (const uint4 *)pc_of(S, b), S.ss(), begun, done, pin ? S.nsys : 0,
+	                      head_first ? DoneSignal{ &S.sf->cnt_head, &S.sf->head_done, S.sync_base + b + 1 } : DoneSignal{}));
 	if (last && !S.flag_sync) *handoff = done;
 	return GF2BV_OK;
 }
@@ -948,7 +972,7 @@
 
 int panel_handover(Solver &S, int b)
 {
-	k_gate<<<dim3(1, S.nsys), dim3(64), 0, S.sA>>>(S.sf, S.st, S.sync_base + b + 1, 0, 0, 0, S.ss());
+	k_gate<<<dim3(1, S.nsys), dim3(64), 0, S.sA>>>(S.sf, S.st, S.sync_base + b + 1, 0, 0, 0, S.ss(), 0, 0, 0);
 	HIPCHK(hipGetLastError());
 	return GF2BV_OK;
 }
@@ -1013,17 +1037,26 @@
 	return GF2BV_OK;
 }
 
-int enqueue_block_bulk(Solver &S, int b)
+int enqueue_block_bulk(Solver &S, int b, bool trsm_early = false, bool head_first = false)
 {
 	const BlockGeom g = block_geom(S, b);
 	if (S.bulk_waits_outer) { HIPCHK(hipStreamWaitEvent(S.sB, S.evOuter, 0)); S.bulk_waits_outer = false; }
+	trsm_early = trsm_early && g.nt_all > 0;
+	if (trsm_early) {
+		k_gate<<<dim3(1, 1), dim3(64), 0, S.sC>>>(S.sf, S.st, 0, 0, S.sync_base + b + 1, 0, S.ss(), 0, 0, S.sync_base + b);
+		int rc = launch_trsm(S, S.sC, b, g.j0, g.gb, g.wlo, g.wlo, g.wlo + g.gnext, true);
+		if (rc) return rc;
+		k_gate<<<dim3(1, 1), dim3(64), 0, S.sC>>>(S.sf, S.st, 0, 0, 0, 0, S.ss(), S.sync_base + b + 1, 0, 0);
+		HIPCHK(hipGetLastError());
+	}
 	if (S.flag_sync) {
-		k_gate<<<dim3(1, S.nsys), dim3(64), 0, S.sB>>>(S.sf, S.st, 0, S.sync_base + b, S.sync_base + b + 1, 0, S.ss());
+		k_gate<<<dim3(1, S.nsys), dim3(64), 0, S.sB>>>(S.sf, S.st, 0, S.sync_base + b, S.sync_base + b + 1, 0, S.ss(),
+		                                               0, trsm_early ? S.sync_base + b + 1 : 0, 0);
 		HIPCHK(hipGetLastError());
 	} else HIPCHK(hipStreamWaitEvent(S.sB, S.evA[b], 0));
 	bool launched = false;
 	if (g.nt_all > 0) {
-		int rc = launch_trsm(S, S.sB, g.j0, g.gb, g.wlo, g.wlo, g.wlo + g.gnext);
+		int rc = trsm_early ? GF2BV_OK : launch_trsm(S, S.sB, b, g.j0, g.gb, g.wlo, g.wlo, g.wlo + g.gnext);
 		if (rc) return rc;
 		const int wend = g.wlo + g.gnext;
 		const int tfull = g.gnext > 0 ? (wend + 1) / 2 : g.wlo / 2;
@@ -1034,9 +1067,10 @@
 			launched = nfull <= 0;
 		}
 		if (nfull > 0) {
-			rc = launch_update_timed(S, S.sB, b, g.j0, g.gb, g.wlo, g.mset, tfull, (int)nfull, 0, true, &S.waitPrio[b]);
+			rc = launch_update_timed(S, S.sB, b, g.j0, g.gb, g.wlo, g.mset, tfull, (int)nfull, 0, true, &S.waitPrio[b], head_first);
 			if (rc) return rc;
 			launched = true;
+			if (head_first) S.head_pass = b;
 		}
 	}
 	if (!launched && !S.flag_sync) {
@@ -1054,7 +1088,7 @@
 	const unsigned row_blocks = (unsigned)((S.rows + 255) / 256);
 	if (b > 0 && !S.flag_sync) HIPCHK(hipStreamWaitEvent(S.sA, S.waitPrio[b - 1], 0));
 	if (b > 0 && S.flag_sync) {
-		k_gate<<<dim3(1, S.nsys), dim3(64), 0, S.sA>>>(S.sf, S.st, 0, 0, 0, S.sync_base + b, S.ss());
+		k_gate<<<dim3(1, S.nsys), dim3(64), 0, S.sA>>>(S.sf, S.st, 0, 0, 0, S.sync_base + b, S.ss(), 0, 0, 0);
 		HIPCHK(hipGetLastError());
 	}
 	k_prio_window<<<dim3(row_blocks, S.nsys), dim3(256), 0, S.sA>>>(S.M, S.rows, S.srows, g.j0, g.gb, g.wlo, std::max(g.gnext, 1),
@@ -1068,6 +1102,7 @@
 {
 	HIPCHK(hipEventRecord(S.ev0, S.sA));
 	HIPCHK(hipStreamWaitEvent(S.sB, S.ev0, 0));
+	if (S.early) HIPCHK(hipStreamWaitEvent(S.sC, S.ev0, 0));
 	if (S.npanels > 0 && gather_first_window) {
 		const int g0 = std::min(S.impl->G, S.npanels);
 		k_win_gather<<<dim3((unsigned)((S.rows * g0 + 255) / 256), S.nsys), dim3(256), 0, S.sA>>>(S.M, S.rows, S.srows, 0, g0, S.Wb, S.st, S.ss());
@@ -1077,6 +1112,10 @@
 
 int enqueue_forward_join(Solver &S)
 {
+	if (S.early) {
+		HIPCHK(hipEventRecord(S.evPri, S.sC));
+		HIPCHK(hipStreamWaitEvent(S.sA, S.evPri, 0));
+	}
 	HIPCHK(hipEventRecord(S.ev3, S.sB));
 	HIPCHK(hipStreamWaitEvent(S.sA, S.ev3, 0));
 	if (S.nblocks > 1 && S.maxr > 0)
@@ -1179,12 +1218,16 @@
 		S.bulk_waits_outer = false;
 		HIPCHK(hipMemsetAsync(&S.st->poison, 0, sizeof(int), S.sA));
 		S.sync_base += S.nblocks + 1;
+		S.head_pass = -1;
 		return GF2BV_OK;
 	};
 	int sparse_probes = 1;
 	auto one_block = [&](int blk) -> int {
 		int r;
 		bool sp = sparse_ok(blk);
+		auto fused_search = [&](int k) { return S.early && k < S.nblocks && optimistic && !sparse_ok(k) && fast_only_ok(k); };
+		const bool trsm_early = blk >= 1 && fused_search(blk) && S.head_pass == blk - 1;
+		const bool head_first = fused_search(blk + 1);
 		if ((r = enqueue_block_panel(S, blk, sp || (optimistic && fast_only_ok(blk)), sp))) return r;
 		if (sp && sparse_probes > 0) {
 			sparse_probes--;
@@ -1199,7 +1242,7 @@
 				if ((r = enqueue_block_panel(S, blk, false, false))) return r;
 			} else S.sparse_tier = std::max(S.sparse_tier, want);
 		}
-		if ((r = enqueue_block_bulk(S, blk))) return r;
+		if ((r = enqueue_block_bulk(S, blk, trsm_early, head_first))) return r;
 		if ((r = enqueue_block_prio(S, blk))) return r;
 		if (blk == 0 && may_probe) {
 			HIPCHK(hipMemcpyAsync(&hst, S.st, sizeof hst, hipMemcpyDeviceToHost, S.sA));
@@ -1402,6 +1445,7 @@
 int solver_enqueue(Solver &S)
 {
 	Trace tr;
+	S.may_early = true;
 	int rc = solver_alloc(S);
 	tr.mark(S.kn, "solver_alloc");
 	if (rc) return rc;
@@ -3287,6 +3331,13 @@
 		hipFuncAttributes a{};
 		HIPCHK(hipFuncGetAttributes(&a, (const void *)k_block_sparse<256, 4>));
 		out[15] = a.numRegs; out[16] = (int32_t)a.sharedSizeBytes;
+	}
+	if (n >= 21) {
+		hipFuncAttributes a{};
+		HIPCHK(hipFuncGetAttributes(&a, (const void *)k_block_trsm<TW, 4, true>));
+		out[17] = a.numRegs; out[18] = (int32_t)a.sharedSizeBytes;
+		HIPCHK(hipFuncGetAttributes(&a, (const void *)k_update16_head_first));
+		out[19] = a.numRegs; out[20] = (int32_t)a.sharedSizeBytes;
 	}
 	return GF2BV_OK;
 	});
diff --git a/gf2bv_amd/hip.py b/gf2bv_amd/hip.py
--- a/gf2bv_amd/hip.py
+++ b/gf2bv_amd/hip.py
@@ -1185,13 +1185,15 @@
 
 
 def kernel_resources(device: int = 0) -> dict:
-    out = (ctypes.c_int32 * 20)()
-    _check(lib().gf2bv_kernel_resources(device, out, 20))
+    out = (ctypes.c_int32 * 24)()
+    _check(lib().gf2bv_kernel_resources(device, out, 24))
     names = ("update", "block_fast", "narrow_all", "prio_window", "panel_step")
     res = {nm: {"vgprs": int(out[2 * k]), "lds": int(out[2 * k + 1])} for k, nm in enumerate(names)}
     res["update_outer"] = {"vgprs": int(out[10]), "lds": int(out[11]), "scratch": int(out[12])}
     res["block_fast_narrow"] = {"vgprs": int(out[13]), "lds": int(out[14])}
     res["block_sparse"] = {"vgprs": int(out[15]), "lds": int(out[16])}
+    res["block_trsm_early"] = {"vgprs": int(out[17]), "lds": int(out[18])}
+    res["update_head_first"] = {"vgprs": int(out[19]), "lds": int(out[20])}
     return res
 
 
```

Result: slower. 7.969 billion (-1.8%).
